# xmed-lab/NEURONS

Measured on AMD Instinct MI355X. Metric: denoising frames/sec, 16f x 256^2 clip, 50 DDIM steps, higher is better.
Workload: dtype bf16; 1 GPU; BASELINE config 2: 1 clip(s) per call, (1,4,16,32,32) latent, 50 DDIM steps, CFG 8.5 (batch 2), SparseCtrl + temporal U-Net per step, random-init weights; clips_per_gpu=5, ddim_steps=50, hip_graph=True, output_finite=True, attention=bf16

## Files before the change

include/neurons_amd.h:

```cpp
#ifndef NEURONS_AMD_H
#define NEURONS_AMD_H

#include <stdint.h>

#ifdef __cplusplus
extern "C" {
#endif

typedef int nr_status;
#define NR_OK 0
#define NR_ERR_ARG 1
#define NR_ERR_STATE 2
#define NR_ERR_MISSING_WEIGHT 3
#define NR_ERR_HIP 4
#define NR_ERR_UNSUPPORTED 5

typedef void* nr_stream;
typedef struct nr_net nr_net;

#define NR_KIND_UNET3D 0
#define NR_KIND_SPARSECTRL 1
#define NR_KIND_SGM_UNET 2

#define NR_KIND_VAE_DECODER 3
// ... 90 lines not shown
                                 double alpha_cumprod_t, double alpha_cumprod_prev, double beta_t);

nr_status nr_cfg_ddim_step(nr_stream stream, const float* eps_dev, const float* x_dev, float* x_out_dev, int64_t n,
                           float guidance_scale, int32_t do_cfg, double alpha_prod_t, double alpha_prod_t_prev);

#define NR_DDIM_EPSILON 0
#define NR_DDIM_SAMPLE 1
#define NR_DDIM_V_PREDICTION 2
nr_status nr_cfg_ddim_step_ex(nr_stream stream, const float* eps_dev, const float* x_dev, float* x_out_dev, float* x0_out_dev, int64_t n,
                              float guidance_scale, int32_t do_cfg, int32_t prediction_type, int32_t clip_sample,
                              int32_t use_clipped_model_output, double alpha_prod_t, double alpha_prod_t_prev, double sigma, double dir_coeff,
                              const float* noise_dev);

nr_status nr_cfg_combine(nr_stream stream, const float* eps_dev, float* eps_out_dev, int64_t n, float guidance_scale);

#define NR_PROF_IGEMM 0
#define NR_PROF_GROUPNORM 1
#define NR_PROF_LAYERNORM 2
#define NR_PROF_ATTENTION 3
#define NR_PROF_OTHER 4
#define NR_PROF_KINDS 5
typedef struct nr_profile {
  double ms[NR_PROF_KINDS];
  double flops[NR_PROF_KINDS];
  double bytes[NR_PROF_KINDS];
  int32_t launches[NR_PROF_KINDS];
} nr_profile;
nr_status nr_net_profile_last(nr_net* h, nr_stream stream, nr_profile* out);

nr_status nr_sparsectrl_forward_async(nr_net* ctrl, nr_stream stream, const float* timesteps, const float* ctx_dev, int32_t ctx_len,
                                      const float* cond_dev, const float* mask_dev, int32_t cond_batch, float scale,
                                      void* const* out_down_dev, void* out_mid_dev, int32_t slot);
nr_status nr_unet3d_forward_after(nr_net* unet, nr_net* ctrl, int32_t slot, nr_stream stream, const float* sample_dev,
                                  const float* timesteps, const float* ctx_dev, int32_t ctx_len, const void* const* down_res_dev,
                                  const void* mid_res_dev, float* out_dev);

nr_status nr_net_set_attention_fp8(nr_net* h, int32_t enable);

nr_status nr_net_set_weight_fp8(nr_net* h, int32_t enable);

nr_status nr_sparsectrl_set_condition_frames(nr_net* h, const int32_t* frames, int32_t n);

nr_status nr_net_set_deterministic_batch(nr_net* h, int32_t enable);
nr_status nr_net_set_clip_samples(nr_net* h, int32_t samples);
nr_status nr_net_set_cfg_pair_identical(nr_net* h, int32_t enable);

int64_t nr_net_export_manifest(nr_net* h, char* buf, int64_t capacity, int64_t* arena_bytes);
nr_status nr_net_export_weights(nr_net* h, nr_stream stream, void* dst_dev, int64_t capacity);
nr_status nr_net_import_weights(nr_net* h, nr_stream stream, const char* manifest, int64_t manifest_bytes, const void* src_dev,
                                int64_t arena_bytes);

nr_status nr_net_set_debug(nr_net* h, int32_t keep_all_activations);
int32_t nr_net_num_taps(const nr_net* h);
const char* nr_net_tap_name(const nr_net* h, int32_t i);
nr_status nr_net_read_tap(nr_net* h, int32_t i, float* host_out, int64_t capacity, int32_t* rows, int32_t* C);

int32_t nr_net_num_ops(const nr_net* h);
const char* nr_net_op_desc(const nr_net* h, int32_t i);

void nr_g8p_set_mode(int32_t mode);
void nr_g8p_set_phases(int32_t phases);
void nr_ff_set_waves(int32_t waves);

nr_status nr_leaf_forward(nr_net* h, nr_stream stream, const float* x_dev, const float* ctx_dev, int32_t ctx_len, float* out_dev);

void nr_op_fm_cache_clear(void);
nr_status nr_op_gemm(nr_stream stream, const void* a_dev, int32_t lda, const void* w_dev, const float* bias_dev,
                     const void* res_dev, int32_t ldr, void* out_dev, int32_t ldo, int32_t M, int32_t N, int32_t K,
                     int32_t geglu);
nr_status nr_op_w8_pack(nr_stream stream, const void* w_dev, int32_t N, int32_t K, void* out_dev, int64_t capacity);
nr_status nr_op_gemm2(nr_stream stream, const void* a0_dev, int32_t c0, int32_t lda0, const void* a1_dev, int32_t c1, int32_t lda1,
                      const void* w_dev, const float* bias_dev, const void* res_dev, int32_t ldr, void* out_dev, int32_t ldo, int32_t M,
                      int32_t N);
nr_status nr_op_ln_gemm(nr_stream stream, const void* a_dev, int32_t lda, const void* w_scaled_dev, const float* ln_c_dev,
                        const float* bias_folded_dev, float eps, const void* res_dev, int32_t ldr, void* out_dev, int32_t ldo,
                        int32_t M, int32_t N, int32_t K, int32_t geglu, int32_t act);
nr_status nr_op_gemm_ex(nr_stream stream, const void* a_dev, int32_t lda, const void* w_dev, const float* bias_dev,
                        const float* ln_c_dev, float ln_eps, const float* rowvec_dev, int32_t rowvec_div, int32_t rowvec_mod,
                        int32_t rowvec_ld, const void* res_dev, int32_t ldr, void* out_dev, int32_t ldo, int32_t M, int32_t N,
                        int32_t K, int32_t geglu, int32_t act, float out_scale);
nr_status nr_op_conv3x3(nr_stream stream, const void* x0_dev, int32_t c0, const void* x1_dev, int32_t c1, int32_t nimg,
                        int32_t H, int32_t W, int32_t stride, int32_t ups, const void* w_dev, const float* bias_dev,
                        const float* rowvec_dev, int32_t rowvec_div, const void* res_dev, void* out_dev, int32_t Cout);
nr_status nr_op_condembed_in(nr_stream stream, const float* cond_dev, const float* mask_dev, int32_t c0, int32_t nsrc, int32_t F, int32_t H,
                             int32_t W, const int32_t* fmap, int32_t nframes, const float* w_dev, const float* bias_dev, int32_t Cout,
                             void* out_dev);
nr_status nr_op_condembed_conv(nr_stream stream, const void* x_dev, int32_t nimg, int32_t H, int32_t W, int32_t Cin, int32_t stride,
                               const void* wfm_dev, const float* bias_dev, int32_t Cout, int32_t silu, void* out_dev);
nr_status nr_op_conv3x3_tap_inner(nr_stream stream, const void* x0, int32_t c0, int32_t nimg, int32_t H, int32_t W, const void* w,
                                  const float* bias, const float* rowvec, int32_t rowvec_div, const void* res, void* out, int32_t Cout);
nr_status nr_op_groupnorm(nr_stream stream, const void* x0_dev, int32_t c0, const void* x1_dev, int32_t c1, int32_t nimg,
                          int32_t hw, int32_t groups, const float* gamma_dev, const float* beta_dev, float eps,
                          int32_t silu, float* partial_ws_dev, void* out_dev);
nr_status nr_op_layernorm(nr_stream stream, const void* x_dev, void* out_dev, int32_t M, int32_t C,
                          const float* gamma_dev, const float* beta_dev, float eps, const float* pe_dev, int32_t pe_hw,
                          int32_t pe_F);
nr_status nr_op_attention(nr_stream stream, int32_t mode, const void* q_dev, const void* kv_dev, void* out_dev,
                          int32_t nimg, int32_t L, int32_t Lk, int32_t C, int32_t heads, int32_t frames, int32_t kv_div);

nr_status nr_op_ff_fused(nr_stream stream, const void* t_dev, const void* x_dev, void* out_dev, int32_t M, int32_t C,
                         const void* w1_geglu_dev, const float* gamma_dev, const float* beta_dev, const float* b1_geglu_dev,
                         const void* wc_dev, const float* bc_dev, float ln_eps);

nr_status nr_op_tattn_fused(nr_stream stream, void* t_dev, int32_t nbatch, int32_t hw, const void* wq_dev, const void* wk_dev,
                            const void* wv_dev, const void* wo_dev, const float* gamma_dev, const float* gb_dev, const float* bo_dev,
                            float ln_eps);
nr_status nr_op_xattn_fused(nr_stream stream, void* t_dev, int32_t nimg, int32_t hw, int32_t img_per_ctx, const void* wq_dev,
                            const void* wo_dev, const void* kv_dev, int32_t ldkv, int32_t Lk, int32_t nctx, const float* gamma_dev,
                            const float* beta_dev, const float* bo_dev, float ln_eps);
nr_status nr_op_tattn_fused_frames(nr_stream stream, void* t_dev, int32_t nbatch, int32_t frames, int32_t hw, const void* wq_dev,
                                   const void* wk_dev, const void* wv_dev, const void* wo_dev, const float* gamma_dev, const float* gb_dev,
                                   const float* bo_dev, float ln_eps);

nr_status nr_op_tattn_head(nr_stream stream, const void* t_dev, void* a_dev, int32_t nbatch, int32_t hw, int32_t C, const void* w_folded_dev,
                           const float* lnc_dev, const float* bias_dev, const float* rowvec_dev, float ln_eps);
nr_status nr_op_tattn_head_frames(nr_stream stream, const void* t_dev, void* a_dev, int32_t nbatch, int32_t frames, int32_t hw, int32_t C,
                                  const void* w_folded_dev, const float* lnc_dev, const float* bias_dev, const float* rowvec_dev, float ln_eps);

nr_status nr_op_xattn_head(nr_stream stream, const void* t_dev, void* a_dev, int32_t nimg, int32_t hw, int32_t img_per_ctx, int32_t C,
                           const void* wq_folded_dev, const float* lnc_dev, const float* bias_dev, const void* kv_dev, int32_t ldkv, int32_t Lk,
                           int32_t nctx, float ln_eps);

#ifdef __cplusplus
}
#endif
#endif
```

neurons_amd/_lib.py:

```python
import ctypes as C
import os

_HERE = os.path.dirname(os.path.abspath(__file__))
LIB_PATH = os.path.join(_HERE, "libneurons_amd" + ("_" + os.environ["NR_LIB_VARIANT"] if os.environ.get("NR_LIB_VARIANT") else "") + ".so")

NR_KIND_UNET3D = 0
NR_KIND_SPARSECTRL = 1
NR_KIND_SGM_UNET = 2
NR_KIND_VAE_DECODER = 3
NR_KIND_VAE_ENCODER = 4
NR_KIND_CLIP_TEXT = 5
NR_KIND_LEAF_TRANSFORMER3D = 6
NR_KIND_LEAF_TEMPORAL = 7
NR_MAX_LEVELS = 4
NR_DDIM_EPSILON = 0
NR_DDIM_SAMPLE = 1
NR_DDIM_V_PREDICTION = 2


class NrNetConfig(C.Structure):
    _fields_ = [
        ("kind", C.c_int32),
        ("in_channels", C.c_int32),
        ("out_channels", C.c_int32),
# ... 11 lines not shown
        ("motion_num_attention_blocks", C.c_int32),
        ("motion_pe_max_len", C.c_int32),
        ("motion_module_mid_block", C.c_int32),
        ("conditioning_channels", C.c_int32),
        ("set_noisy_sample_input_to_zero", C.c_int32),
        ("transformer_depth", C.c_int32 * NR_MAX_LEVELS),
        ("num_head_channels", C.c_int32),
        ("adm_in_channels", C.c_int32),
        ("cond_embedding_levels", C.c_int32),
        ("cond_embedding_channels", C.c_int32 * NR_MAX_LEVELS),
    ]


NR_PROF_KINDS = 5
NR_PROF_NAMES = ("igemm", "groupnorm", "layernorm", "attention", "other")


class NrProfile(C.Structure):
    _fields_ = [("ms", C.c_double * NR_PROF_KINDS), ("flops", C.c_double * NR_PROF_KINDS),
                ("bytes", C.c_double * NR_PROF_KINDS), ("launches", C.c_int32 * NR_PROF_KINDS)]


_VP = C.c_void_p
_FP = C.POINTER(C.c_float)
_I32 = C.c_int32
_I64 = C.c_int64
SYMBOLS = {
    "nr_net_create": (_I32, [C.POINTER(NrNetConfig), C.POINTER(_VP)]),
    "nr_net_destroy": (None, [_VP]),
    "nr_last_error": (C.c_char_p, []),
    "nr_net_load_tensor": (_I32, [_VP, C.c_char_p, _VP, C.POINTER(_I64), _I32]),
    "nr_net_plan": (_I32, [_VP, _I32, _I32, _I32, _I32, _I32]),
    "nr_net_release_host_weights": (_I32, [_VP]),
    "nr_net_invalidate_context": (_I32, [_VP]),
    "nr_net_set_graph": (_I32, [_VP, _I32]),
    "nr_net_workspace_bytes": (_I64, [_VP]),
    "nr_net_weight_bytes": (_I64, [_VP]),
    "nr_net_num_residuals": (_I32, [_VP]),
    "nr_net_residual_shape": (_I32, [_VP, _I32, C.POINTER(_I32), C.POINTER(_I32), C.POINTER(_I32)]),
    "nr_unet3d_forward": (_I32, [_VP, _VP, _VP, _FP, _VP, _I32, C.POINTER(_VP), _VP, _VP]),
    "nr_sparsectrl_forward": (_I32, [_VP, _VP, _VP, _FP, _VP, _I32, _VP, _VP, _I32, C.c_float, C.POINTER(_VP), _VP]),
    "nr_denoise_step_forward": (_I32, [_VP, _VP, _VP, _VP, _FP, _VP, _I32, _VP, _VP, _I32, C.c_float, C.POINTER(_VP), _VP, _VP, _FP]),
    "nr_sparsectrl_forward_async": (_I32, [_VP, _VP, _FP, _VP, _I32, _VP, _VP, _I32, C.c_float, C.POINTER(_VP), _VP, _I32]),
    "nr_unet3d_forward_after": (_I32, [_VP, _VP, _I32, _VP, _VP, _FP, _VP, _I32, C.POINTER(_VP), _VP, _VP]),
    "nr_sgm_unet_forward": (_I32, [_VP, _VP, _VP, C.c_float, _FP, _VP, _I32, _VP, _VP]),
    "nr_vae_decode": (_I32, [_VP, _VP, _VP, C.c_float, C.c_float, C.c_float, _I32, _VP]),
    "nr_clip_text_forward": (_I32, [_VP, _VP, _VP, _VP]),
    "nr_vae_encode": (_I32, [_VP, _VP, _VP, C.c_float, C.c_float, _VP]),
    "nr_gaussian_sample": (_I32, [_VP, _VP, _VP, _VP, _I32, _I32, _I32, C.c_float]),
    "nr_edm_cfg_euler_step": (_I32, [_VP, _VP, _VP, _VP, _I64, C.c_float, C.c_float, C.c_float, C.c_float]),
    "nr_prior_p_sample_step": (_I32, [_VP, _VP, _VP, _VP, _VP, _VP, _VP, _I64, C.c_float, _I32, _I32, C.c_double, C.c_double, C.c_double]),
    "nr_cfg_ddim_step": (_I32, [_VP, _VP, _VP, _VP, _I64, C.c_float, _I32, C.c_double, C.c_double]),
    "nr_cfg_ddim_step_ex": (_I32, [_VP, _VP, _VP, _VP, _VP, _I64, C.c_float, _I32, _I32, _I32, _I32, C.c_double, C.c_double, C.c_double,
                                   C.c_double, _VP]),
    "nr_cfg_combine": (_I32, [_VP, _VP, _VP, _I64, C.c_float]),
    "nr_net_export_manifest": (_I64, [_VP, _VP, _I64, C.POINTER(_I64)]),
    "nr_net_export_weights": (_I32, [_VP, _VP, _VP, _I64]),
    "nr_net_import_weights": (_I32, [_VP, _VP, C.c_char_p, _I64, _VP, _I64]),
    "nr_net_profile_last": (_I32, [_VP, _VP, C.POINTER(NrProfile)]),
    "nr_net_set_attention_fp8": (_I32, [_VP, _I32]),
    "nr_net_set_weight_fp8": (_I32, [_VP, _I32]),
    "nr_net_set_deterministic_batch": (_I32, [_VP, _I32]),
    "nr_net_set_clip_samples": (_I32, [_VP, _I32]),
    "nr_net_set_cfg_pair_identical": (_I32, [_VP, _I32]),
    "nr_sparsectrl_set_condition_frames": (_I32, [_VP, C.POINTER(_I32), _I32]),
    "nr_net_set_debug": (_I32, [_VP, _I32]),
    "nr_net_num_taps": (_I32, [_VP]),
    "nr_net_tap_name": (C.c_char_p, [_VP, _I32]),
    "nr_net_read_tap": (_I32, [_VP, _I32, _VP, _I64, C.POINTER(_I32), C.POINTER(_I32)]),
    "nr_g8p_set_mode": (None, [_I32]),
    "nr_g8p_set_phases": (None, [_I32]),
    "nr_ff_set_waves": (None, [_I32]),
    "nr_net_num_ops": (_I32, [_VP]),
    "nr_net_op_desc": (C.c_char_p, [_VP, _I32]),
    "nr_leaf_forward": (_I32, [_VP, _VP, _VP, _VP, _I32, _VP]),
    "nr_op_fm_cache_clear": (None, []),
    "nr_op_gemm": (_I32, [_VP, _VP, _I32, _VP, _VP, _VP, _I32, _VP, _I32, _I32, _I32, _I32, _I32]),
    "nr_op_w8_pack": (_I32, [_VP, _VP, _I32, _I32, _VP, _I64]),
    "nr_op_gemm2": (_I32, [_VP, _VP, _I32, _I32, _VP, _I32, _I32, _VP, _VP, _VP, _I32, _VP, _I32, _I32, _I32]),
    "nr_op_ln_gemm": (_I32, [_VP, _VP, _I32, _VP, _VP, _VP, C.c_float, _VP, _I32, _VP, _I32, _I32, _I32, _I32, _I32, _I32]),
    "nr_op_gemm_ex": (_I32, [_VP, _VP, _I32, _VP, _VP, _VP, C.c_float, _VP, _I32, _I32, _I32, _VP, _I32, _VP, _I32, _I32, _I32, _I32, _I32, _I32,
                             C.c_float]),
    "nr_op_conv3x3": (_I32, [_VP, _VP, _I32, _VP, _I32, _I32, _I32, _I32, _I32, _I32, _VP, _VP, _VP, _I32, _VP, _VP, _I32]),
    "nr_op_condembed_in": (_I32, [_VP, _VP, _VP, _I32, _I32, _I32, _I32, _I32, C.POINTER(_I32), _I32, _VP, _VP, _I32, _VP]),
    "nr_op_condembed_conv": (_I32, [_VP, _VP, _I32, _I32, _I32, _I32, _I32, _VP, _VP, _I32, _I32, _VP]),
    "nr_op_conv3x3_tap_inner": (_I32, [_VP, _VP, _I32, _I32, _I32, _I32, _VP, _VP, _VP, _I32, _VP, _VP, _I32]),
    "nr_op_groupnorm": (_I32, [_VP, _VP, _I32, _VP, _I32, _I32, _I32, _I32, _VP, _VP, C.c_float, _I32, _VP, _VP]),
    "nr_op_layernorm": (_I32, [_VP, _VP, _VP, _I32, _I32, _VP, _VP, C.c_float, _VP, _I32, _I32]),
    "nr_op_attention": (_I32, [_VP, _I32, _VP, _VP, _VP, _I32, _I32, _I32, _I32, _I32, _I32, _I32]),
    "nr_op_ff_fused": (_I32, [_VP, _VP, _VP, _VP, _I32, _I32, _VP, _VP, _VP, _VP, _VP, _VP, C.c_float]),
    "nr_op_tattn_fused": (_I32, [_VP, _VP, _I32, _I32, _VP, _VP, _VP, _VP, _VP, _VP, _VP, C.c_float]),
    "nr_op_xattn_fused": (_I32, [_VP, _VP, _I32, _I32, _I32, _VP, _VP, _VP, _I32, _I32, _I32, _VP, _VP, _VP, C.c_float]),
    "nr_op_tattn_fused_frames": (_I32, [_VP, _VP, _I32, _I32, _I32, _VP, _VP, _VP, _VP, _VP, _VP, _VP, C.c_float]),
    "nr_op_tattn_head": (_I32, [_VP, _VP, _VP, _I32, _I32, _I32, _VP, _VP, _VP, _VP, C.c_float]),
    "nr_op_tattn_head_frames": (_I32, [_VP, _VP, _VP, _I32, _I32, _I32, _I32, _VP, _VP, _VP, _VP, C.c_float]),
    "nr_op_xattn_head": (_I32, [_VP, _VP, _VP, _I32, _I32, _I32, _I32, _VP, _VP, _VP, _VP, _I32, _I32, _I32, C.c_float]),
}

_lib = None


def load():
    global _lib
    if _lib is not None:
        return _lib
    if not os.path.exists(LIB_PATH):
        raise RuntimeError(
            f"{LIB_PATH} not found: build it with `python -c 'import __graft_entry__ as g; g.build()'` "
            "(make -C neurons_amd/csrc).  neurons_amd has no CPU fallback."
        )
    lib = C.CDLL(LIB_PATH)
    for name, (res, args) in SYMBOLS.items():
        fn = getattr(lib, name)
        fn.restype = res
        fn.argtypes = args
    _lib = lib
    return lib


def check(status):
    if status != 0:
        msg = load().nr_last_error()
        raise RuntimeError(f"neurons_amd: status {status}: {msg.decode() if msg else ''}")
```

neurons_amd/csrc/common.h:

```cpp
#pragma once
#include <hip/hip_runtime.h>
#include <stdint.h>
#include <cmath>
#include <cstring>

typedef __bf16 bf16;
typedef __attribute__((ext_vector_type(8))) __bf16 bf16x8;
typedef __attribute__((ext_vector_type(4))) __bf16 bf16x4;
typedef __attribute__((ext_vector_type(2))) __bf16 bf16x2;
typedef __attribute__((ext_vector_type(4))) float f32x4;

#define NR_WAVE 64

__device__ __forceinline__ float bf2f(bf16 v) { return (float)v; }
__device__ __forceinline__ bf16 f2bf(float v) { return (bf16)v; }

__device__ __forceinline__ bf16x8 bf16x8_zero() {
  bf16x8 z;
#pragma unroll
  for (int i = 0; i < 8; ++i) z[i] = (bf16)0.0f;
  return z;
}

__device__ __forceinline__ float silu_f(float x) { return x * __builtin_amdgcn_rcpf(1.0f + __expf(-x)); }
// ... 76 lines not shown
  p.out_f32 = nr_pin(p.out_f32); p.tap_inner = nr_pin(p.tap_inner); p.w_fm = nr_pin(p.w_fm); p.w8 = nr_pin(p.w8);
  return p;
}

struct NrRowPanelParams {
  const bf16* a; int lda;
  const bf16* w;
  int M, N;
  const float* bias;
  const float* ln_c; float ln_eps;
  const float* rowvec; int rowvec_div, rowvec_mod, rowvec_ld;
  const bf16* res; int ldr;
  bf16* out; int ldo;
  float out_scale; int geglu; int act;
  int nsplit;
};

struct NrAttnParams {
  const bf16* q; const bf16* k; const bf16* v; bf16* out;
  long long q_outer, q_inner_stride, q_seq;
  long long kv_outer, kv_inner_stride, kv_seq;
  long long o_outer, o_inner_stride, o_seq;
  int inner;
  int kv_inner;
  int kv_div;
  int nbatch, heads, d, Lq, Lk;
  float scale;
  int causal;
  int fp8;
};

struct NrGnParams {
  const bf16* x0; const bf16* x1;
  int c0, c1, ld0, ld1;
  int nimg, hw;
  int plan_nimg;
  int groups;
  int pix_per_blk, nchunk;
  float* partial;
  int finalized;
  const float* gamma; const float* beta;
  float eps;
  int silu;
  bf16* out; int ldo;
};

struct NrFfFusedParams {
  const bf16* t; int ldt; const bf16* x; int ldx; bf16* out; int ldo; int M; const bf16* stream; const float *gamma, *beta, *b1, *bc; float ln_eps; int norot, waves; };
struct NrXattnFusedParams {
  bf16* t; int nimg, hw, img_per_ctx, nctx, Lk; const bf16* wstream; const bf16* kvstream; const float *gamma, *beta, *bo; float ln_eps; int norot; };
struct NrTattnFusedParams {
  bf16* t; int nbatch, frames, hw; const bf16* stream; const float *gamma, *gb, *bo; float ln_eps; int norot; };
struct NrXattnHeadParams {
  const bf16* t; bf16* out; int nimg, hw, img_per_ctx, nctx, Lk, C; const bf16* wstream; const bf16* kvstream; const float* table; float ln_eps; };
struct NrTattnHeadParams {
  const bf16* t; bf16* out; int nbatch, frames, hw, C; const bf16* stream; const float* table; float ln_eps; };

struct NrAddMulti {
  bf16* dst[16];
  const bf16* src[16];
  long long n8_end[16];
  int count;
};


inline void nr_conv_out_hw(int H, int W, int ksize, int stride, int ups, int* OH, int* OW) {
  *OH = H; *OW = W;
  if (ksize == 3) {
    if (ups) { *OH *= 2; *OW *= 2; }
    if (stride == 2) { *OH = (*OH - 1) / 2 + 1; *OW = (*OW - 1) / 2 + 1; }
  }
}

inline NrGemmParams nr_gemm_params(const bf16* a0, int c0, int lda0, const bf16* a1, int c1, int lda1, int nimg, int H, int W, int ksize, int stride,
                                   int ups, const bf16* w, int N, const float* bias, const bf16* res, int ldr, bf16* out, int ldo) {
  NrGemmParams p;
  std::memset(&p, 0, sizeof(p));
  p.a0 = a0; p.c0 = c0; p.lda0 = lda0;
  p.a1 = a1; p.c1 = a1 ? c1 : 0; p.lda1 = lda1;
  p.H = H; p.W = W;
  nr_conv_out_hw(H, W, ksize, stride, ups, &p.OH, &p.OW);
  p.ksize = ksize; p.stride = stride; p.ups = ups;
  p.w = w;
  p.M = nimg * p.OH * p.OW; p.N = N; p.K = ksize * ksize * (p.c0 + p.c1);
  p.bias = bias; p.rowvec_div = 1;
  p.res = res; p.ldr = ldr;
  p.out = out; p.ldo = ldo; p.out_scale = 1.f;
  return p;
}

inline NrAttnParams nr_attn_params(int mode, const bf16* q, const bf16* kv, bf16* out, int ldq, int ldkv, int ldo, int nimg, int hw, int Lk, int C,
                                   int heads, int frames, int kv_div, int causal, int fp8) {
  NrAttnParams p;
  std::memset(&p, 0, sizeof(p));
  p.heads = heads; p.d = C / heads; p.scale = 1.0f / std::sqrt((float)p.d);
  p.out = out; p.causal = causal; p.fp8 = fp8;
  if (mode == 0) {
    p.q = q; p.k = q + C; p.v = q + 2 * C;
    p.nbatch = nimg; p.Lq = hw; p.Lk = hw;
    p.inner = 1; p.q_outer = (long long)hw * ldq; p.q_inner_stride = 0; p.q_seq = ldq;
    p.kv_inner = 1; p.kv_outer = p.q_outer; p.kv_inner_stride = 0; p.kv_seq = ldq; p.kv_div = 1;
    p.o_outer = (long long)hw * ldo; p.o_inner_stride = 0; p.o_seq = ldo;
  } else if (mode == 1) {
    p.q = q; p.k = kv; p.v = kv + C;
    p.nbatch = nimg; p.Lq = hw; p.Lk = Lk;
    p.inner = 1; p.q_outer = (long long)hw * ldq; p.q_inner_stride = 0; p.q_seq = ldq;
    p.kv_inner = 1; p.kv_outer = (long long)Lk * ldkv; p.kv_inner_stride = 0; p.kv_seq = ldkv; p.kv_div = kv_div;
    p.o_outer = (long long)hw * ldo; p.o_inner_stride = 0; p.o_seq = ldo;
  } else {
    const int F = frames;
    p.q = q; p.k = q + C; p.v = q + 2 * C;
    p.nbatch = (nimg / F) * hw; p.Lq = F; p.Lk = F;
    p.inner = hw; p.q_outer = (long long)F * hw * ldq; p.q_inner_stride = ldq; p.q_seq = (long long)hw * ldq;
    p.kv_inner = hw; p.kv_outer = p.q_outer; p.kv_inner_stride = ldq; p.kv_seq = p.q_seq; p.kv_div = 1;
    p.o_outer = (long long)F * hw * ldo; p.o_inner_stride = ldo; p.o_seq = (long long)hw * ldo;
  }
  return p;
}

inline NrGnParams nr_gn_params(const bf16* x0, int c0, int ld0, const bf16* x1, int c1, int ld1, int nimg, int hw, int groups, const float* gamma,
                               const float* beta, float eps, int silu, float* partial, bf16* out, int ldo) {
  NrGnParams p;
  std::memset(&p, 0, sizeof(p));
  p.x0 = x0; p.c0 = c0; p.ld0 = ld0;
  p.x1 = x1; p.c1 = x1 ? c1 : 0; p.ld1 = ld1;
  p.nimg = nimg; p.hw = hw; p.groups = groups; p.partial = partial;
  p.gamma = gamma; p.beta = beta; p.eps = eps; p.silu = silu;
  p.out = out; p.ldo = ldo;
  return p;
}
```

neurons_amd/csrc/engine.h:

```cpp
#pragma once
#include "launchers.h"
#include "../../include/neurons_amd.h"

#include <algorithm>
#include <cmath>
#include <cstdio>
#include <cstdlib>
#include <cstring>
#include <functional>
#include <map>
#include <memory>
#include <stdexcept>
#include <string>
#include <vector>

namespace nre {

void set_err(const std::string& s);

struct NrError : std::runtime_error {
  nr_status code;
  NrError(nr_status c, const std::string& m) : std::runtime_error(m), code(c) {}
};

#define HIP_OK(expr)                                                                                        \
  do {                                                                                                      \
    hipError_t _e = (expr);                                                                                 \
    if (_e != hipSuccess) throw nre::NrError(NR_ERR_HIP, std::string(#expr) + ": " + hipGetErrorString(_e)); \
  } while (0)

#define LAUNCH_OK(expr)                                                                                   \
  do {                                                                                                    \
    int _r = (expr);                                                                                      \
    if (_r != 0) throw nre::NrError(NR_ERR_UNSUPPORTED, std::string(#expr) + " -> " + std::to_string(_r)); \
    hipError_t _le = hipGetLastError();                                                                   \
    if (_le != hipSuccess) throw nre::NrError(NR_ERR_HIP, std::string(#expr) + ": " + hipGetErrorString(_le)); \
  } while (0)

#define NR_TRY try {
#define NR_CATCH                                                                   \
  }                                                                                \
  catch (const nre::NrError& e) { nre::set_err(e.what()); return e.code; }         \
  catch (const std::exception& e) { nre::set_err(e.what()); return NR_ERR_STATE; } \
  return NR_OK;

inline float bf2f_host(uint16_t h) {
  const uint32_t u = (uint32_t)h << 16;
  float f;
  std::memcpy(&f, &u, 4);
  return f;
}
inline uint16_t f2bf_host(float f) {
  uint32_t u;
  std::memcpy(&u, &f, 4);
  if ((u & 0x7fffffffu) > 0x7f800000u) return 0x7fc0;
  u += 0x7fffu + ((u >> 16) & 1u);
  return (uint16_t)(u >> 16);
}

template <class... A>
std::string descf(const char* fmt, A... a) { char d[160]; snprintf(d, sizeof(d), fmt, a...); return d; }
inline bool env_is_1(const char* name) {
  const char* v = getenv(name);
  return v && v[0] == '1';
}

struct HostTensor {
  std::vector<float> data;
  std::vector<int64_t> shape;
  int64_t numel() const { int64_t n = 1; for (auto s : shape) n *= s; return n; }
};

struct Arena {
  struct Blk { size_t off, size; };
  std::vector<Blk> free_;
  size_t top = 0, high = 0;
  static size_t align(size_t b) { return (b + 255) & ~(size_t)255; }
  size_t alloc(size_t bytes);
  void release(size_t off, size_t bytes);
  void reset() { free_.clear(); top = 0; high = 0; }
};

struct Buf {
  Arena* arena; size_t off, bytes; bool keep;
  ~Buf() { if (!keep) arena->release(off, bytes); }
};

struct Act {
  std::shared_ptr<Buf> buf;
  bf16* ptr = nullptr;
  int nimg = 0, H = 0, W = 0, C = 0, ld = 0;
  int64_t rows() const { return (int64_t)nimg * H * W; }
  bool valid() const { return nimg > 0; }
};

struct Tap { std::string name; bf16* ptr; int64_t rows; int C, ld; };

struct IO {
  const float* sample;
  const float* ctx;
  float* out;
  const void* down_res[16];
  const void* mid_res;
  int has_res;
  const float* cond;
  const float* mask;
  int cond_batch;
  float scale;
  void* out_down[16];
  void* out_mid;
  const float* y;
  float in_scale;
  const int* ids;
  float in_shift;
  float out_mul, out_add;
  int clamp01;
  bool operator==(const IO& o) const { return std::memcmp(this, &o, sizeof(IO)) == 0; }
};
inline IO new_io() {
  IO io;
  std::memset(&io, 0, sizeof(io));
  io.scale = 1.f; io.in_scale = 1.f; io.out_mul = 1.f; io.cond_batch = 1;
  return io;
}

constexpr int NR_MAX_BATCH = 64;

void launch_copy16(const void* src, void* dst, size_t nbytes, hipStream_t s);

struct TembSlot { std::string prefix; int off, C; };

std::vector<float> sinusoid_table(int max_len, int C);

struct WeightStore {
  const bool& dry;
  explicit WeightStore(const bool& sizing_pass) : dry(sizing_pass) {}
  ~WeightStore();
  WeightStore(const WeightStore&) = delete;

  std::map<std::string, HostTensor> host;
  struct DevW { void* ptr; size_t bytes; };
  std::map<std::string, DevW> dev;
  size_t weight_bytes = 0;
  char* import_base = nullptr;
  size_t import_bytes = 0;
  bool in_import(const void* p) const { return import_base && (const char*)p >= import_base && (const char*)p < import_base + import_bytes; }

  bool load_tensor(const std::string& key, const float* data, const int64_t* shape, int ndim);
  void release_host();
  const HostTensor& need(const std::string& key) const;
  bool has(const std::string& key) const { return host.count(key) != 0; }
  const HostTensor& data_of(const std::string& key) const;
  void check_shape(const std::string& key, const HostTensor& t, std::initializer_list<int64_t> want) const;

  std::string manifest(int kind, size_t* total) const;
  void export_to(void* dst_dev, hipStream_t s) const;
  void import_from(int kind, const std::string& manifest, const void* src_dev, int64_t arena_bytes, hipStream_t s);

  void* upload(const std::string& name, const void* data, size_t bytes);
  void* adopt(const std::string& name, void* d, size_t bytes);
  void erase(const std::string& name);
  std::string name_of(const void* p, const char* who) const;
  template <class Fn>
  void* cached(const std::string& name, Fn make) {
    if (dry) return nullptr;
    auto it = dev.find(name);
    if (it != dev.end()) return it->second.ptr;
    return make();
  }
  template <class Fn>
  void* packed(const std::string& name, size_t bytes, Fn fn, const std::vector<std::string>& inputs = {}) {
    return cached(name, [&]() {
      std::vector<char> had;
      for (auto& in : inputs) had.push_back(dev.count(in) != 0);
      void* d = nullptr;
      HIP_OK(hipMalloc(&d, bytes));
      try { fn(d); HIP_OK(hipDeviceSynchronize()); }
      catch (...) { (void)hipFree(d); throw; }
      adopt(name, d, bytes);
      for (size_t i = 0; i < inputs.size(); ++i) if (!had[i]) erase(inputs[i]);
      return d;
    });
  }
  template <class T, class Fill>
  const T* convert(const char* tag, const std::string& key, std::initializer_list<int64_t> shape, size_t count, Fill fill) {
    check_shape(key, need(key), shape);
    const std::string name = tag + key;
    return (const T*)cached(name, [&]() {
      const HostTensor& t = data_of(key);
      std::vector<T> h(count);
      fill(t.data.data(), h.data());
      return upload(name, h.data(), h.size() * sizeof(T));
    });
  }
  template <class T, class Cvt>
  const T* stacked(const std::string& name, const std::vector<std::string>& keys, Cvt cvt) {
    return (const T*)cached(name, [&]() {
      std::vector<T> h;
      for (auto& k : keys) { const HostTensor& t = data_of(k); for (float f : t.data) h.push_back(cvt(f)); }
      return upload(name, h.data(), h.size() * sizeof(T));
    });
  }

  const bf16* w_linear(const std::string& key, int N, int K);
  const bf16* w_linear_cat(const std::vector<std::string>& keys, int Neach, int K);
  const float* b_cat(const std::vector<std::string>& keys, int Neach);
  struct Stacked { const bf16* w; const float* b; };
  Stacked w_temb_projection(const std::string& tag, const std::vector<TembSlot>& slots, const std::string& layer, int K);
  struct LnW { const bf16* w; const float* c; const float* b; };
  LnW w_ln_linear(const std::vector<std::string>& wkeys, const std::vector<std::string>& bkeys, const std::string& ln, int Neach, int K, bool geglu);
  const float* pe_projection(const std::vector<std::string>& wkeys, int Neach, int K, int max_len);
  struct FoldW { const bf16* w; const float* b; };
  FoldW w_fold_ff_proj(const std::string& ff2, const std::string& po, int C);
  const bf16* w_geglu(const std::string& key, int inner, int K);
  const float* b_geglu(const std::string& key, int inner);
  const bf16* w_conv3(const std::string& key, int Cout, int Cin, bool tap_inner = false);
  const float* w_conv_in(const std::string& key, int Cout, int Cin);
  const bf16* w_condembed(const std::string& key, int Cout, int Cin);
  const float* w_f32_sum(const std::string& a, const std::string& b, int64_t n);
  const float* w_f32(const std::string& key, std::initializer_list<int64_t> shape);
  const float* w_f32(const std::string& key, int64_t n) { return w_f32(key, {n}); }
  const float* pe_table(int C, int max_len);
  const float* b_ln_pe(const std::string& ln, int F, int C);
  const bf16* w_layout(const bf16* w, int N, int K, int layout);

  struct FfFusedW { const bf16* stream; const float *gamma, *beta, *b1, *bc; };
  FfFusedW ff_fused_weights(const std::string& ln, const std::string& ff, const std::string& po, int C);
  struct XattnFusedW { const bf16* wstream; const float *gamma, *beta, *bo; };
  XattnFusedW xattn_fused_weights(const std::string& b, int C);
  struct TattnFusedW { const bf16* stream; const float *gb, *gamma, *bo; };
  TattnFusedW tattn_fused_weights(const std::string& ln, const std::string& ab, int F, int C);
  struct HeadW { const bf16* stream; const float* table; };
  HeadW xattn_head_weights(const std::string& ln, const std::string& wq, int C);
  HeadW tattn_head_weights(const std::string& ln, const std::vector<std::string>& wqkv, int C, int F, int max_len);
  LnW ln_vectors(const std::vector<std::string>& wkeys, const std::string& ln, int Neach, int K);
  const float* fold_bias(const std::string& ff2, const std::string& po, int C);
};

}

struct nr_net {
  using Arena = nre::Arena;
  using Buf = nre::Buf;
  using Act = nre::Act;
  using IO = nre::IO;
  static constexpr int NR_MAX_BATCH = nre::NR_MAX_BATCH;

  nr_net_config cfg;
  int device = -1;

  int B2 = 0, F = 0, H = 0, W = 0, ctx_len = 0;
  bool planned = false;
  bool dry = false;
  nre::WeightStore wts{dry};
  Arena arena;
  Arena parena;
  size_t main_high = 0;
  char* arena_base = nullptr;
  size_t arena_bytes = 0;
  std::vector<std::function<void(hipStream_t)>> ops;
  std::vector<std::function<void(hipStream_t)>> ctx_ops;
  std::vector<Act> ctx_persist;
  bool building_ctx = false;
  bool ctx_dirty = true;
  struct OpMeta { int kind; double flops, bytes; std::string desc; int launches = 1; };
  std::vector<OpMeta> op_meta;
  std::vector<nre::Tap> taps;
  bool keep_all = false;
  bool det_batch = false;
  int clip_samples = 2;
  long long det_rows(long long rows) const {
    if (!det_batch || B2 <= clip_samples) return rows;
    return rows / B2 * clip_samples;
  }
  int n_cond_frames = -1;
  int cond_frames[64] = {0};
  bool cfg_dup = false;
  bool attn_fp8 = false;
  bool w8 = false;
  IO io = nre::new_io();
  int n_res = 0;
  struct ResShape { int C, h, w; };
  std::vector<ResShape> res_shapes;

  float* t_dev = nullptr;
  int temb_total = 0;

  bool use_graph = false;
  struct GraphSlot { IO io = nre::new_io(); hipGraphExec_t exec = nullptr; unsigned long long used = 0; };
  static constexpr int NR_GRAPH_SLOTS = 64;
  std::vector<GraphSlot> gcache[3];
  unsigned long long gclock = 0;
  hipEvent_t ev_slot[2] = {nullptr, nullptr};
  size_t split_op = 0;
  size_t split_op2 = 0;
  hipEvent_t ev_adds = nullptr;
  bool prefetch_valid = false;
  float prefetch_t[NR_MAX_BATCH] = {0};
  IO prefetch_io = nre::new_io();
  hipStream_t own_stream = nullptr;
  hipEvent_t ev_in = nullptr, ev_out = nullptr;

  ~nr_net();

  template <class T>
  T* at(size_t off) const { return reinterpret_cast<T*>(reinterpret_cast<uintptr_t>(arena_base) + off); }
  Act new_act(int nimg, int h, int w, int C) { return act_in(arena, 0, keep_all, nimg, h, w, C); }
  Act new_act_persistent(int nimg, int h, int w, int C) { return act_in(parena, main_high, true, nimg, h, w, C); }
  Act act_in(Arena& a, size_t base, bool keep, int nimg, int h, int w, int C);
  template <class T>
  T* new_scratch(size_t count) { return at<T>(arena.alloc(count * sizeof(T))); }
  std::shared_ptr<Buf> new_tmp(size_t bytes);
  struct SplitK { std::shared_ptr<Buf> buf; float* ws = nullptr; };
  SplitK splitk_scratch(size_t bytes);
  void emit(std::function<void(hipStream_t)> fn, int kind = NR_PROF_OTHER, double flops = 0, double bytes = 0, const std::string& desc = std::string());
  void last_op_launches(int n) { if (!dry && !building_ctx && !op_meta.empty()) op_meta.back().launches = n; }
  void tap(const std::string& name, const Act& a) {
    if (!dry && keep_all) taps.push_back(nre::Tap{name, a.ptr, a.rows(), a.C, a.ld});
  }
  void op_tap(const char* kind, const Act& a);
  void begin_plan();
  Act stage_context();
  Act context_kv(const Act& ctx_bf, const std::string& b, int C, size_t stream_bytes = 0, const std::function<void(const bf16*, int, bf16*, hipStream_t)>& pack = nullptr);

  struct GemmOpt {
    const float* bias = nullptr;
    const float* rowvec = nullptr; int rowvec_div = 1, rowvec_ld = 0, rowvec_mod = 0;
    const Act* res = nullptr;
    float scale = 1.f;
    int geglu = 0;
    Act* out = nullptr;
    int pad_tl0 = 0;
    int act = 0;
    const float* ln_c = nullptr;
    int tap_inner = 0;
    bool derived_w = false;
  };
  Act conv(const Act& x0, const Act* x1, const bf16* w, int Cout, int ksize, int stride, int ups, const GemmOpt& o);
  Act linear(const Act& x, const bf16* w, int N, const GemmOpt& o) { return conv(x, nullptr, w, N, 1, 1, 0, o); }
  Act linear_wb(const Act& x, const std::string& key, int N, const Act* res = nullptr, Act* out = nullptr);
  void gemm_raw(const bf16* a, int lda, const bf16* w, int M, int N, int K, const float* bias, bf16* out, int ldo, float* out32, const char* what);
  Act groupnorm(const Act& x0, const Act* x1, const std::string& prefix, float eps, int silu);
  Act layernorm(const Act& x, const std::string& prefix, const float* pe, int pe_F);
  Act attention(int mode, const Act& q, const Act* kv, int C, int heads, int causal = 0);
  using TembSlot = nre::TembSlot;
  std::vector<TembSlot> temb_slots;
  float* temb_all = nullptr;
  const float* temb_for(const std::string& prefix, int C);
  struct ResKeys { std::string norm1, conv1, norm2, conv2, shortcut; };
  ResKeys res_keys(const std::string& pre) const;
  Act resnet(const Act& x0, const Act* x1, const std::string& pre, int Cout);
  Act ln_linear(const Act& x, const std::string& ln, const std::vector<std::string>& wkeys, const std::vector<std::string>& bkeys, int Neach, bool geglu,
                int act, bool temporal_pe);
  void feed_forward(Act& t, const std::string& ln, const std::string& pre);
  Act feed_forward_proj_out(const Act& x, Act& t, const std::string& ln, const std::string& ff, const std::string& pre);
  bool cfg_dedup_active() const;
  Act expand_cfg(const Act& h);
  enum BlockKernel { BLOCK_UNFUSED, BLOCK_FUSED320, BLOCK_HEAD };
  BlockKernel cross_attn_kernel(const Act& t, int heads, int hw) const;
  BlockKernel temporal_attn_kernel(const Act& t, int heads, int hw) const;
  Act ff_fused_block(const Act& x, const Act& t, const std::string& ln, const std::string& ff, const std::string& po);
  void xattn_fused_block(Act& t, const Act& ctx_bf, const std::string& b, int hw);
  Act xattn_head_block(const Act& t, const Act& ctx_bf, const std::string& b, int hw);
  void tattn_fused_block(Act& t, const std::string& nrm, const std::string& ab, int hw, int heads);
  Act tattn_head_block(const Act& t, const std::string& nrm, const std::vector<std::string>& wqkv, int hw, int heads);
  Act spatial_transformer(const Act& x_in, const Act& ctx_bf, const std::string& pre, int depth = 1, bool cfg_half = false, Act* x_full = nullptr);
  Act temporal_module(const Act& x, const std::string& pre0);
  Act vae_attn(const Act& x, const std::string& pre);

  void enumerate_resnets(std::vector<TembSlot>& out) const;
  struct SgmLayout {
    struct In { int idx; int kind; int level; int Cout; };
    struct Out { int idx; int level; int Cout; bool attn; bool up; };
    std::vector<In> in;
    std::vector<Out> out;
  };
  SgmLayout sgm_layout() const;
  void build_sgm();
  void build_vae();
  void build_vae_enc();
  void build_clip();
  void build_leaf();
  Act embed_conv(const Act& in, int Fe, const std::string& key, int Cout, int stride, int silu, const float* bias);
  void cond_embedding(Act& x, int nd, const int* fmap_reduce, const int* fmap_expand);
  void build();
  void plan(int batch, int frames, int h, int w, int ctxl);

  void drop_graphs();
  void ensure_streams();
  void run_context(hipStream_t s);
  void set_timesteps(hipStream_t s, const float* timesteps);
  void launch_segment(hipStream_t s, int seg);
  void begin(hipStream_t s, const float* timesteps) { set_timesteps(s, timesteps); run_context(s); }
  void run_eager(hipStream_t s, const float* timesteps);
  hipStream_t begin_fenced(hipStream_t caller, const float* timesteps);
  void run(hipStream_t caller, const float* timesteps);
};
```

neurons_amd/csrc/engine_layers.hip:

```cpp
#include "engine.h"

using namespace nre;

size_t Arena::alloc(size_t bytes) {
  bytes = align(bytes);
  for (size_t i = 0; i < free_.size(); ++i) {
    if (free_[i].size >= bytes) {
      const size_t off = free_[i].off;
      if (free_[i].size == bytes) free_.erase(free_.begin() + i);
      else { free_[i].off += bytes; free_[i].size -= bytes; }
      return off;
    }
  }
  const size_t off = top;
  top += bytes;
  if (top > high) high = top;
  return off;
}
void Arena::release(size_t off, size_t bytes) {
  bytes = align(bytes);
  size_t i = 0;
  while (i < free_.size() && free_[i].off < off) ++i;
  free_.insert(free_.begin() + i, Blk{off, bytes});
  if (i + 1 < free_.size() && free_[i].off + free_[i].size == free_[i + 1].off) {
    free_[i].size += free_[i + 1].size;
    free_.erase(free_.begin() + i + 1);
  }
  if (i > 0 && free_[i - 1].off + free_[i - 1].size == free_[i].off) {
    free_[i - 1].size += free_[i].size;
    free_.erase(free_.begin() + i);
  }
  if (!free_.empty() && free_.back().off + free_.back().size == top) {
    top = free_.back().off;
    free_.pop_back();
  }
}

Act nr_net::act_in(Arena& ar, size_t base, bool keep, int nimg, int h, int w, int C) {
  Act a;
  const size_t bytes = (size_t)nimg * h * w * C * sizeof(bf16);
  auto b = std::make_shared<Buf>();
  b->arena = &ar; b->bytes = bytes; b->off = ar.alloc(bytes); b->keep = keep;
  a.buf = b; a.ptr = at<bf16>(base + b->off); a.nimg = nimg; a.H = h; a.W = w; a.C = C; a.ld = C;
  return a;
}
std::shared_ptr<Buf> nr_net::new_tmp(size_t bytes) {
  auto b = std::make_shared<Buf>();
  b->arena = &arena; b->bytes = bytes; b->off = arena.alloc(bytes); b->keep = keep_all;
  return b;
}
nr_net::SplitK nr_net::splitk_scratch(size_t bytes) {
  SplitK k;
  if (bytes) { k.buf = new_tmp(bytes); k.ws = at<float>(k.buf->off); }
  return k;
}
void nr_net::emit(std::function<void(hipStream_t)> fn, int kind, double flops, double bytes, const std::string& desc) {
  if (dry) return;
  if (building_ctx) { ctx_ops.push_back(std::move(fn)); return; }
  ops.push_back(std::move(fn));
  op_meta.push_back(OpMeta{kind, flops, bytes, desc});
}
void nr_net::op_tap(const char* kind, const Act& a) {
  static const bool on = getenv("NR_OP_TAPS") != nullptr;
  if (on && !dry && keep_all && !building_ctx) taps.push_back(Tap{"op" + std::to_string(ops.size()) + "." + kind, a.ptr, a.rows(), a.C, a.ld});
}
void nr_net::begin_plan() {
  ctx_persist.clear(); ops.clear(); ctx_ops.clear(); op_meta.clear(); taps.clear(); arena.reset(); parena.reset();
  ctx_dirty = true;
  temb_slots.clear(); temb_total = 0; temb_all = nullptr;
  n_res = 0; res_shapes.clear();
  t_dev = new_scratch<float>(NR_MAX_BATCH);
}
Act nr_net::stage_context() {
  Act ctx_bf = new_act_persistent(1, 1, B2 * ctx_len, cfg.cross_attention_dim);
  bf16* cp = ctx_bf.ptr; const long long n = (long long)B2 * ctx_len * cfg.cross_attention_dim;
  building_ctx = true;
  emit([this, cp, n](hipStream_t s) { LAUNCH_OK(nr_launch_f32_to_bf16(io.ctx, cp, n, s)); });
  building_ctx = false;
  ctx_persist.push_back(ctx_bf);
  return ctx_bf;
}
Act nr_net::context_kv(const Act& ctx_bf, const std::string& b, int C, size_t stream_bytes, const std::function<void(const bf16*, int, bf16*, hipStream_t)>& pack) {
  building_ctx = true;
  Act kv = new_act_persistent(ctx_bf.nimg, ctx_bf.H, ctx_bf.W, 2 * C);
  GemmOpt ok; ok.out = &kv;
  linear(ctx_bf, wts.w_linear_cat({b + ".attn2.to_k.weight", b + ".attn2.to_v.weight"}, C, cfg.cross_attention_dim), 2 * C, ok);
  Act stream;
  if (pack) {
    stream = new_act_persistent(1, 1, 1, (int)(stream_bytes / sizeof(bf16)));
    const bf16* kvp = kv.ptr; bf16* sp = stream.ptr; const int ldkv = kv.ld;
    emit([=](hipStream_t s) { pack(kvp, ldkv, sp, s); });
  }
  building_ctx = false;
  ctx_persist.push_back(kv);
  if (pack) ctx_persist.push_back(stream);
  return pack ? stream : kv;
}

Act nr_net::conv(const Act& x0, const Act* x1, const bf16* w, int Cout, int ksize, int stride, int ups, const GemmOpt& o) {
  int OH, OW;
  nr_conv_out_hw(x0.H, x0.W, ksize, stride, ups, &OH, &OW);
  const int outC = o.geglu ? Cout / 2 : Cout;
  Act out = o.out ? *o.out : new_act(x0.nimg, OH, OW, outC);
  if (out.C != outC || out.rows() != (int64_t)x0.nimg * OH * OW) throw NrError(NR_ERR_STATE, "conv: output shape mismatch");
  if (o.res && (o.res->C != outC || o.res->rows() != out.rows())) throw NrError(NR_ERR_STATE, "conv: residual shape mismatch");
  NrGemmParams p = nr_gemm_params(x0.ptr, x0.C, x0.ld, x1 ? x1->ptr : nullptr, x1 ? x1->C : 0, x1 ? x1->ld : 0, x0.nimg, x0.H, x0.W, ksize, stride, ups,
                                  w, Cout, o.bias, o.res ? o.res->ptr : nullptr, o.res ? o.res->ld : 0, out.ptr, out.ld);
  p.rowvec = o.rowvec; p.rowvec_div = o.rowvec_div; p.rowvec_ld = o.rowvec_ld; p.rowvec_mod = o.rowvec_mod;
  p.out_scale = o.scale; p.geglu = o.geglu; p.pad_tl0 = o.pad_tl0; p.act = o.act; p.ln_c = o.ln_c; p.ln_eps = 1e-5f;
  p.tap_inner = o.tap_inner;
  p.plan_m = det_batch ? (int)det_rows(p.M) : 0;
  p.w8 = (w8 && ksize == 1 && !o.derived_w) ? 1 : 0;
  NrGemmRoute r;
  LAUNCH_OK(nr_gemm_route(&p, &r));
  const bf16* wk = dry ? reinterpret_cast<const bf16*>(uintptr_t(16)) : wts.w_layout(w, Cout, p.K, r.weight_layout);
  const double in_elems = (double)x0.rows() * (p.c0 + p.c1);
  const double bytes = 2.0 * (in_elems + (double)p.N * p.K + (double)p.M * outC + (o.res ? (double)p.M * outC : 0.0));
  const bool l160 = r.cls == NR_GEMM_LIN160;
  const std::string d = l160 ? descf("%s M=%d N=%d K=%d res=%d geglu=%d ln=%d", r.lin160.form == 4 ? "lin160 panel" : "lin160", p.M, p.N, p.K, o.res ? 1 : 0, p.geglu, p.ln_c ? 1 : 0)
                             : descf("igemm ks=%d s=%d ups=%d M=%d N=%d K=%d geglu=%d res=%d%s", ksize, stride, ups, p.M, p.N, p.K, p.geglu, o.res ? 1 : 0,
                                     r.weight_layout == NR_W_FRAGMAJOR_E4M3 ? " w=e4m3" : "");
  const SplitK sk = splitk_scratch(r.ws_bytes);
  float* ws = sk.ws;
  emit([p, r, wk, ws](hipStream_t s) { LAUNCH_OK(nr_launch_gemm(&p, &r, wk, ws, s)); }, NR_PROF_IGEMM, 2.0 * p.M * (double)p.N * p.K, bytes, d);
  if (ws) last_op_launches(2);
  op_tap(l160 ? "lin160" : (ksize == 3 ? "conv3" : (p.ln_c ? "lngemm" : "gemm")), out);
  return out;
}

Act nr_net::linear_wb(const Act& x, const std::string& key, int N, const Act* res, Act* out) {
  GemmOpt o; o.bias = wts.w_f32(key + ".bias", N); o.res = res; o.out = out;
  return linear(x, wts.w_linear(key + ".weight", N, x.C), N, o);
}

void nr_net::gemm_raw(const bf16* a, int lda, const bf16* w, int M, int N, int K, const float* bias, bf16* out, int ldo, float* out32,
                      const char* what) {
  NrGemmParams p = nr_gemm_params(a, K, lda, nullptr, 0, 0, M, 1, 1, 1, 1, 0, w, N, bias, nullptr, 0, out, ldo);
  p.out_f32 = out32;
  p.plan_m = det_batch ? (int)det_rows(M) : 0;
  NrGemmRoute r;
  LAUNCH_OK(nr_gemm_route_rowmajor(&p, &r));
  const SplitK sk = splitk_scratch(r.ws_bytes);
  float* ws = sk.ws;
  emit([p, r, ws](hipStream_t s) { LAUNCH_OK(nr_launch_gemm(&p, &r, p.w, ws, s)); }, NR_PROF_IGEMM, 2.0 * M * (double)N * K,
       2.0 * ((double)M * K + (double)N * K) + (out32 ? 4.0 : 2.0) * (double)M * N, descf("igemm %s M=%d N=%d K=%d", what, M, N, K));
}

Act nr_net::groupnorm(const Act& x0, const Act* x1, const std::string& prefix, float eps, int silu) {
  const int C = x0.C + (x1 ? x1->C : 0);
  const float* gamma = wts.w_f32(prefix + ".weight", C);
  const float* beta = wts.w_f32(prefix + ".bias", C);
  NrGnParams p = nr_gn_params(x0.ptr, x0.C, x0.ld, x1 ? x1->ptr : nullptr, x1 ? x1->C : 0, x1 ? x1->ld : 0, x0.nimg, x0.H * x0.W, cfg.norm_num_groups, gamma, beta,
                              eps, silu, nullptr, nullptr, C);
  if (x1) p.c1 = x1->C;
  p.plan_nimg = det_batch ? (int)det_rows(x0.nimg) : 0;
  NrGnRoute r;
  LAUNCH_OK(nr_gn_route(&p, &r));
  auto ws = new_tmp((size_t)r.ws_floats * sizeof(float));
  Act out = new_act(x0.nimg, x0.H, x0.W, C);
  p.partial = at<float>(ws->off); p.out = out.ptr;
  if (getenv("NR_OP_TAPS") && keep_all && !x1) {
    Act snap = new_act(x0.nimg, x0.H, x0.W, x0.C);
    const bf16* src = x0.ptr; bf16* dst = snap.ptr; const size_t nb = (size_t)x0.rows() * x0.C * sizeof(bf16);
    if (x0.ld == x0.C) {
      emit([=](hipStream_t s) { launch_copy16(src, dst, nb, s); });
      op_tap("gn_input_snapshot", snap);
    }
  }
  emit([p, r](hipStream_t s) { LAUNCH_OK(nr_launch_groupnorm(&p, &r, s)); }, NR_PROF_GROUPNORM,
       8.0 * (double)x0.rows() * C, 2.0 * 2.0 * (double)x0.rows() * C,
       "groupnorm nimg=" + std::to_string(x0.nimg) + " hw=" + std::to_string(x0.H * x0.W) + " C=" + std::to_string(C));
  last_op_launches(r.launches);
  op_tap("gn", out);
  return out;
}

Act nr_net::layernorm(const Act& x, const std::string& prefix, const float* pe, int pe_F) {
  const float* g = wts.w_f32(prefix + ".weight", x.C);
  const float* b = wts.w_f32(prefix + ".bias", x.C);
  Act out = new_act(x.nimg, x.H, x.W, x.C);
  const bf16* xp = x.ptr; bf16* op = out.ptr;
  const int ldx = x.ld, ldo = out.ld, M = (int)x.rows(), C = x.C, hw = x.H * x.W;
  emit([=](hipStream_t s) { LAUNCH_OK(nr_launch_layernorm(xp, ldx, op, ldo, M, C, g, b, 1e-5f, pe, hw, pe_F, s)); },
       NR_PROF_LAYERNORM, 8.0 * (double)M * C, 2.0 * 2.0 * (double)M * C,
       "layernorm M=" + std::to_string(M) + " C=" + std::to_string(C));
  op_tap("ln", out);
  return out;
}

Act nr_net::attention(int mode, const Act& q, const Act* kv, int C, int heads, int causal) {
  Act out = new_act(q.nimg, q.H, q.W, C);
  const bool vae = cfg.kind == NR_KIND_VAE_DECODER || cfg.kind == NR_KIND_VAE_ENCODER;
  const NrAttnParams p = nr_attn_params(mode, q.ptr, kv ? kv->ptr : nullptr, out.ptr, q.ld, kv ? kv->ld : 0, out.ld, q.nimg, q.H * q.W, ctx_len, C, heads, F,
                                        F, causal, (attn_fp8 && mode != 2 && !vae) ? 1 : 0);
  NrAttnRoute r;
  LAUNCH_OK(nr_attn_route(&p, &r));
  const double flops = 4.0 * (double)p.nbatch * p.heads * (double)p.Lq * p.Lk * p.d;
  const double kvrows = mode == 1 ? (double)(p.nbatch / p.kv_div) * p.Lk : (double)p.nbatch * p.Lk;
  const double bytes = 2.0 * ((double)p.nbatch * p.Lq * C * 2.0 + kvrows * C * 2.0);
  emit([p, r](hipStream_t s) { LAUNCH_OK(nr_launch_attention(&p, &r, s)); }, NR_PROF_ATTENTION, flops, bytes,
       descf("attention mode=%d nbatch=%d heads=%d d=%d Lq=%d Lk=%d", mode, p.nbatch, p.heads, p.d, p.Lq, p.Lk));
  op_tap(mode == 2 ? "tattn" : (mode == 1 ? "xattn" : "sattn"), out);
  return out;
}

const float* nr_net::temb_for(const std::string& prefix, int C) {
  for (auto& s : temb_slots) if (s.prefix == prefix) {
    if (s.C != C) throw NrError(NR_ERR_STATE, "temb slot size mismatch for " + prefix);
    return temb_all + s.off;
  }
// ... 306 lines not shown
```

neurons_amd/csrc/engine_nets.hip:

```cpp
#include "engine.h"

using namespace nre;

void nr_net::enumerate_resnets(std::vector<TembSlot>& out) const {
  int off = 0;
  auto add = [&](const std::string& p, int C) { out.push_back(TembSlot{p, off, C}); off += C; };
  const int L = cfg.num_levels;
  for (int i = 0; i < L; ++i)
    for (int j = 0; j < cfg.layers_per_block; ++j)
      add("down_blocks." + std::to_string(i) + ".resnets." + std::to_string(j), cfg.block_out_channels[i]);
  add("mid_block.resnets.0", cfg.block_out_channels[L - 1]);
  add("mid_block.resnets.1", cfg.block_out_channels[L - 1]);
  if (cfg.kind == NR_KIND_UNET3D)
    for (int i = 0; i < L; ++i)
      for (int j = 0; j < cfg.layers_per_block + 1; ++j)
        add("up_blocks." + std::to_string(i) + ".resnets." + std::to_string(j), cfg.block_out_channels[L - 1 - i]);
}

nr_net::SgmLayout nr_net::sgm_layout() const {
  SgmLayout l;
  const int L = cfg.num_levels;
  int idx = 0;
  l.in.push_back({idx++, 0, 0, cfg.block_out_channels[0]});
  for (int lev = 0; lev < L; ++lev) {
// ... 16 lines not shown
  if (F != 1) throw NrError(NR_ERR_ARG, "sgm UNetModel is a 2-D network: plan with frames = 1");
  const SgmLayout lay = sgm_layout();
  begin_plan();
  {
    int off = 0;
    auto add = [&](const std::string& p, int C) { temb_slots.push_back(TembSlot{p, off, C}); off += C; };
    for (auto& b : lay.in) if (b.kind == 1) add("input_blocks." + std::to_string(b.idx) + ".0", b.Cout);
    add("middle_block.0", cfg.block_out_channels[L - 1]);
    add("middle_block.2", cfg.block_out_channels[L - 1]);
    for (auto& b : lay.out) add("output_blocks." + std::to_string(b.idx) + ".0", b.Cout);
    temb_total = off;
  }
  float* sincos = new_scratch<float>((size_t)B2 * C0);
  float* e1 = new_scratch<float>((size_t)B2 * temb_dim);
  float* et = new_scratch<float>((size_t)B2 * temb_dim);
  float* y1 = new_scratch<float>((size_t)B2 * temb_dim);
  float* emb = new_scratch<float>((size_t)B2 * temb_dim);
  temb_all = new_scratch<float>((size_t)B2 * temb_total);
  {
    const int adm = cfg.adm_in_channels;
    const bf16* w1 = wts.w_linear("time_embed.0.weight", temb_dim, C0);
    const float* b1 = wts.w_f32("time_embed.0.bias", temb_dim);
    const bf16* w2 = wts.w_linear("time_embed.2.weight", temb_dim, temb_dim);
    const float* b2 = wts.w_f32("time_embed.2.bias", temb_dim);
    const bf16* wy1 = wts.w_linear("label_emb.0.0.weight", temb_dim, adm);
    const float* by1 = wts.w_f32("label_emb.0.0.bias", temb_dim);
    const bf16* wy2 = wts.w_linear("label_emb.0.2.weight", temb_dim, temb_dim);
    const float* by2 = wts.w_f32("label_emb.0.2.bias", temb_dim);
    const auto proj = wts.w_temb_projection("sgm", temb_slots, ".emb_layers.1", temb_dim);
    const bf16* wp = proj.w; const float* bp = proj.b;
    float* td = t_dev; float* ta = temb_all;
    const int b2n = B2, tt = temb_total;
    emit([=, this](hipStream_t s) {
      LAUNCH_OK(nr_launch_timestep_sincos(td, b2n, C0, sincos, s));
      LAUNCH_OK(nr_launch_linear_small(sincos, b2n, C0, w1, b1, temb_dim, 0, 1, e1, nullptr, s));
      LAUNCH_OK(nr_launch_linear_small(e1, b2n, temb_dim, w2, b2, temb_dim, 0, 0, et, nullptr, s));
      LAUNCH_OK(nr_launch_linear_small(io.y, b2n, adm, wy1, by1, temb_dim, 0, 1, y1, nullptr, s));
      LAUNCH_OK(nr_launch_linear_small(y1, b2n, temb_dim, wy2, by2, temb_dim, 0, 1, emb, et, s));
      LAUNCH_OK(nr_launch_linear_small(emb, b2n, temb_dim, wp, bp, tt, 0, 0, ta, nullptr, s));
    });
    last_op_launches(6);
  }
  Act ctx_bf = stage_context();
  std::vector<Act> hs;
  Act x;
  for (auto& b : lay.in) {
    const std::string bp = "input_blocks." + std::to_string(b.idx);
    if (b.kind == 0) {
      x = new_act(nimg, H, W, C0);
      const float* wT = wts.w_conv_in(bp + ".0.weight", C0, cfg.in_channels);
      const float* bi = wts.w_f32(bp + ".0.bias", C0);
      bf16* xp = x.ptr; const int ic = cfg.in_channels, b2n = B2, Hn = H, Wn = W;
      emit([=, this](hipStream_t s) {
        LAUNCH_OK(nr_launch_conv_in_small(io.sample, nullptr, ic, 0, b2n, nimg, 1, Hn, Wn, wT, bi, nullptr, C0, xp, io.in_scale, 0.f, s));
      });
      tap(bp, x);
    } else if (b.kind == 1) {
      x = resnet(x, nullptr, bp + ".0", b.Cout);
      if (cfg.down_block_has_attn[b.level]) x = spatial_transformer(x, ctx_bf, bp + ".1", cfg.transformer_depth[b.level]);
    } else {
      GemmOpt o; o.bias = wts.w_f32(bp + ".0.op.bias", b.Cout);
      x = conv(x, nullptr, wts.w_conv3(bp + ".0.op.weight", b.Cout, b.Cout), b.Cout, 3, 2, 0, o);
      tap(bp, x);
    }
    hs.push_back(x);
  }
  {
    const int Cm = cfg.block_out_channels[L - 1];
    x = resnet(x, nullptr, "middle_block.0", Cm);
    x = spatial_transformer(x, ctx_bf, "middle_block.1", cfg.transformer_depth[L - 1]);
    x = resnet(x, nullptr, "middle_block.2", Cm);
  }
  for (auto& b : lay.out) {
    const std::string bp = "output_blocks." + std::to_string(b.idx);
    Act skip = hs.back();
    hs.pop_back();
    x = resnet(x, &skip, bp + ".0", b.Cout);
    skip = Act();
    int sub = 1;
    if (b.attn) { x = spatial_transformer(x, ctx_bf, bp + ".1", cfg.transformer_depth[b.level]); sub = 2; }
    if (b.up) {
      const std::string up = bp + "." + std::to_string(sub) + ".conv";
      GemmOpt o; o.bias = wts.w_f32(up + ".bias", b.Cout);
      x = conv(x, nullptr, wts.w_conv3(up + ".weight", b.Cout, b.Cout), b.Cout, 3, 1, 1, o);
      tap(bp + "." + std::to_string(sub), x);
    }
  }
  Act hn = groupnorm(x, nullptr, "out.0", cfg.norm_eps, 1);
  {
    const bf16* wo = wts.w_conv3("out.2.weight", cfg.out_channels, C0);
    const float* bo = wts.w_f32("out.2.bias", cfg.out_channels);
    const bf16* hp = hn.ptr; const int Hn = H, Wn = W, oc = cfg.out_channels;
    emit([=, this](hipStream_t s) { LAUNCH_OK(nr_launch_conv_out_small(hp, C0, nimg, 1, Hn, Wn, wo, bo, oc, io.out, 1.f, 0.f, 0, s)); });
  }
}

void nr_net::build_vae() {
  const int L = cfg.num_levels, zc = cfg.in_channels, nimg = B2;
  if (F != 1) throw NrError(NR_ERR_ARG, "the VAE decoder is a 2-D network: plan with frames = 1");
  begin_plan();
  const int Cm = cfg.block_out_channels[L - 1];
  float* zq = new_scratch<float>((size_t)nimg * zc * H * W);
  {
    const float* Q = wts.w_f32("post_quant_conv.weight", {zc, zc});
    const float* qb = wts.w_f32("post_quant_conv.bias", zc);
    const int hw = H * W;
    emit([=, this](hipStream_t s) { LAUNCH_OK(nr_launch_post_quant(io.sample, io.in_scale, Q, qb, zq, nimg, zc, hw, s)); });
  }
  Act x = new_act(nimg, H, W, Cm);
  {
    const float* wT = wts.w_conv_in("decoder.conv_in.weight", Cm, zc);
    const float* bi = wts.w_f32("decoder.conv_in.bias", Cm);
    bf16* xp = x.ptr; const int Hn = H, Wn = W;
    emit([=](hipStream_t s) {
      LAUNCH_OK(nr_launch_conv_in_small(zq, nullptr, zc, 0, nimg, nimg, 1, Hn, Wn, wT, bi, nullptr, Cm, xp, 1.f, 0.f, s));
    });
    tap("decoder.conv_in", x);
  }
  x = resnet(x, nullptr, "decoder.mid.block_1", Cm);
  x = vae_attn(x, "decoder.mid.attn_1");
  x = resnet(x, nullptr, "decoder.mid.block_2", Cm);
  for (int lev = L - 1; lev >= 0; --lev) {
    const int Co = cfg.block_out_channels[lev];
    const std::string up = "decoder.up." + std::to_string(lev);
    for (int j = 0; j < cfg.layers_per_block + 1; ++j) x = resnet(x, nullptr, up + ".block." + std::to_string(j), Co);
    if (lev != 0) {
      GemmOpt o; o.bias = wts.w_f32(up + ".upsample.conv.bias", Co);
      x = conv(x, nullptr, wts.w_conv3(up + ".upsample.conv.weight", Co, Co), Co, 3, 1, 1, o);
      tap(up + ".upsample", x);
    }
  }
  Act hn = groupnorm(x, nullptr, "decoder.norm_out", cfg.norm_eps, 1);
  {
    const int C0 = cfg.block_out_channels[0], oc = cfg.out_channels;
    const bf16* wo = wts.w_conv3("decoder.conv_out.weight", oc, C0);
    const float* bo = wts.w_f32("decoder.conv_out.bias", oc);
    const bf16* hp = hn.ptr; const int Hn = x.H, Wn = x.W;
    emit([=, this](hipStream_t s) { LAUNCH_OK(nr_launch_conv_out_small(hp, C0, nimg, 1, Hn, Wn, wo, bo, oc, io.out, io.out_mul, io.out_add, io.clamp01, s)); });
  }
}


void nr_net::build_vae_enc() {
  const int L = cfg.num_levels, zc2 = cfg.out_channels, nimg = B2, ic = cfg.in_channels;
  if (F != 1) throw NrError(NR_ERR_ARG, "the VAE encoder is a 2-D network: plan with frames = 1");
  begin_plan();
  const int C0 = cfg.block_out_channels[0];
  Act x = new_act(nimg, H, W, C0);
  {
    const float* wT = wts.w_conv_in("encoder.conv_in.weight", C0, ic);
    const float* bi = wts.w_f32("encoder.conv_in.bias", C0);
    bf16* xp = x.ptr; const int Hn = H, Wn = W;
    emit([=, this](hipStream_t s) {
      LAUNCH_OK(nr_launch_conv_in_small(io.sample, nullptr, ic, 0, nimg, nimg, 1, Hn, Wn, wT, bi, nullptr, C0, xp, io.in_scale,
                                        io.in_shift, s));
    });
    tap("encoder.conv_in", x);
  }
  for (int lev = 0; lev < L; ++lev) {
    const int Co = cfg.block_out_channels[lev];
    const std::string dn = "encoder.down." + std::to_string(lev);
    for (int j = 0; j < cfg.layers_per_block; ++j) x = resnet(x, nullptr, dn + ".block." + std::to_string(j), Co);
    if (lev != L - 1) {
      GemmOpt o; o.bias = wts.w_f32(dn + ".downsample.conv.bias", Co); o.pad_tl0 = 1;
      x = conv(x, nullptr, wts.w_conv3(dn + ".downsample.conv.weight", Co, Co), Co, 3, 2, 0, o);
      tap(dn + ".downsample", x);
    }
  }
  const int Cm = cfg.block_out_channels[L - 1];
  x = resnet(x, nullptr, "encoder.mid.block_1", Cm);
  x = vae_attn(x, "encoder.mid.attn_1");
  x = resnet(x, nullptr, "encoder.mid.block_2", Cm);
  Act hn = groupnorm(x, nullptr, "encoder.norm_out", cfg.norm_eps, 1);
  {
    const int hw = x.H * x.W;
    float* mraw = new_scratch<float>((size_t)nimg * zc2 * hw);
    const bf16* wo = wts.w_conv3("encoder.conv_out.weight", zc2, Cm);
    const float* bo = wts.w_f32("encoder.conv_out.bias", zc2);
    const float* Q = wts.w_f32("quant_conv.weight", {zc2, zc2});
    const float* qb = wts.w_f32("quant_conv.bias", zc2);
    const bf16* hp = hn.ptr; const int Hn = x.H, Wn = x.W;
    emit([=, this](hipStream_t s) {
      LAUNCH_OK(nr_launch_conv_out_small(hp, Cm, nimg, 1, Hn, Wn, wo, bo, zc2, mraw, 1.f, 0.f, 0, s));
      LAUNCH_OK(nr_launch_post_quant(mraw, 1.f, Q, qb, io.out, nimg, zc2, hw, s));
    });
  }
}


void nr_net::build_clip() {
  const int C = cfg.block_out_channels[0], heads = cfg.num_heads, inter = cfg.cross_attention_dim, vocab = cfg.in_channels;
  const int L = W, M = B2 * L;
  if (F != 1 || H != 1) throw NrError(NR_ERR_ARG, "CLIP text encoder: plan with frames = 1, h = 1, w = sequence length");
  if (L > cfg.motion_pe_max_len) throw NrError(NR_ERR_ARG, "sequence longer than max_position_embeddings");
  begin_plan();
  const std::string tm = "text_model.";
  Act x = new_act(B2, 1, L, C);
  {
    const std::string tk = tm + "embeddings.token_embedding.weight", pk = tm + "embeddings.position_embedding.weight";
    const float* tok = wts.w_f32(tk, {vocab, C});
    const float* pos = wts.w_f32(pk, {cfg.motion_pe_max_len, C});
    bf16* xp = x.ptr;
    emit([=, this](hipStream_t s) { LAUNCH_OK(nr_launch_clip_embed(io.ids, tok, pos, xp, M, L, C, vocab, s)); });
    tap("text_model.embeddings", x);
  }
  for (int i = 0; i < cfg.layers_per_block; ++i) {
    const std::string lp = tm + "encoder.layers." + std::to_string(i);
    const std::string ap = lp + ".self_attn";
    Act qkv = ln_linear(x, lp + ".layer_norm1", {ap + ".q_proj.weight", ap + ".k_proj.weight", ap + ".v_proj.weight"},
                        {ap + ".q_proj.bias", ap + ".k_proj.bias", ap + ".v_proj.bias"}, C, false, 0, false);
    Act ao = attention(0, qkv, nullptr, C, heads, 1);
// ... 262 lines not shown
  {
    const int Cm = cfg.block_out_channels[L - 1];
    x = resnet(x, nullptr, "mid_block.resnets.0", Cm);
    x = spatial_transformer(x, ctx_bf, "mid_block.attentions.0");
    if (cfg.use_motion_module && cfg.motion_module_mid_block) x = temporal_module(x, "mid_block.motion_modules.0");
    x = resnet(x, nullptr, "mid_block.resnets.1", Cm);
  }
  res_shapes.push_back(ResShape{x.C, x.H, x.W});
  mid_in = Act();

  if (cfg.kind == NR_KIND_SPARSECTRL) {
    for (int i = 0; i <= n_res; ++i) {
      const bool is_mid = i == n_res;
      const Act& src = is_mid ? x : skips[i];
      const std::string key = is_mid ? std::string("controlnet_mid_block") : "controlnet_down_blocks." + std::to_string(i);
      const bf16* w = wts.w_linear(key + ".weight", src.C, src.C);
      const float* bias = wts.w_f32(key + ".bias", src.C);
      NrGemmParams p = nr_gemm_params(src.ptr, src.C, src.ld, nullptr, 0, 0, src.nimg, src.H, src.W, 1, 1, 0, w, src.C, bias, nullptr, 0, nullptr, src.C);
      p.plan_m = det_batch ? (int)det_rows(p.M) : 0;
      NrGemmRoute r;
      LAUNCH_OK(nr_gemm_route_rowmajor(&p, &r));
      const SplitK sk = splitk_scratch(r.ws_bytes);
      float* ws = sk.ws;
      emit([this, p, r, i, is_mid, ws](hipStream_t s) {
        NrGemmParams q = p;
        q.out = (bf16*)(is_mid ? io.out_mid : io.out_down[i]);
        q.out_scale = io.scale;
        LAUNCH_OK(nr_launch_gemm(&q, &r, q.w, ws, s));
      }, NR_PROF_IGEMM, 2.0 * p.M * (double)p.N * p.K, 2.0 * (2.0 * p.M * (double)p.N + (double)p.N * p.K));
    }
    return;
  }

  split_op = ops.size();
  {
    struct AddT { bf16* dst; long long n; };
    std::vector<AddT> adds;
    for (int i = 0; i < n_res; ++i) adds.push_back(AddT{skips[i].ptr, (long long)skips[i].rows() * skips[i].C});
    adds.push_back(AddT{x.ptr, (long long)x.rows() * x.C});
    bool multi = (int)adds.size() <= 16;
    for (auto& a : adds) multi = multi && a.n % 8 == 0;
    if (multi) {
      NrAddMulti am;
      std::memset(&am, 0, sizeof(am));
      long long acc = 0;
      for (size_t i = 0; i < adds.size(); ++i) { am.dst[i] = adds[i].dst; acc += adds[i].n / 8; am.n8_end[i] = acc; }
      am.count = (int)adds.size();
      const int nr = n_res;
      emit([this, am, nr](hipStream_t st) {
        if (!io.has_res) return;
        NrAddMulti q = am;
        for (int i = 0; i < nr; ++i) q.src[i] = (const bf16*)io.down_res[i];
        q.src[nr] = (const bf16*)io.mid_res;
        LAUNCH_OK(nr_launch_add_bf16_multi(&q, st));
      });
    } else {
      for (int i = 0; i < n_res; ++i) {
        bf16* sp = adds[i].dst; const long long n = adds[i].n;
        emit([this, sp, n, i](hipStream_t st) {
          if (io.has_res) LAUNCH_OK(nr_launch_add_bf16(sp, (const bf16*)io.down_res[i], sp, n, st));
        });
      }
      bf16* xp = x.ptr; const long long n = adds.back().n;
      emit([this, xp, n](hipStream_t st) {
        if (io.has_res) LAUNCH_OK(nr_launch_add_bf16(xp, (const bf16*)io.mid_res, xp, n, st));
      });
    }
  }
  split_op2 = ops.size();

  for (int i = 0; i < L; ++i) {
    const int Cout = cfg.block_out_channels[L - 1 - i];
    const std::string bp = "up_blocks." + std::to_string(i);
    for (int j = 0; j < cfg.layers_per_block + 1; ++j) {
      Act skip = skips.back();
      skips.pop_back();
      x = resnet(x, &skip, bp + ".resnets." + std::to_string(j), Cout);
      skip = Act();
      if (cfg.up_block_has_attn[i]) x = spatial_transformer(x, ctx_bf, bp + ".attentions." + std::to_string(j));
      if (cfg.use_motion_module) x = temporal_module(x, bp + ".motion_modules." + std::to_string(j));
    }
    if (i != L - 1) {
      GemmOpt o; o.bias = wts.w_f32(bp + ".upsamplers.0.conv.bias", Cout);
      x = conv(x, nullptr, wts.w_conv3(bp + ".upsamplers.0.conv.weight", Cout, Cout), Cout, 3, 1, 1, o);
      tap(bp + ".upsamplers.0", x);
    }
  }

  Act hn = groupnorm(x, nullptr, "conv_norm_out", cfg.norm_eps, 1);
  {
    const bf16* wo = wts.w_conv3("conv_out.weight", cfg.out_channels, C0);
    const float* bo = wts.w_f32("conv_out.bias", cfg.out_channels);
    const bf16* hp = hn.ptr; const int Fn = F, Hn = H, Wn = W, oc = cfg.out_channels;
    emit([=, this](hipStream_t s) { LAUNCH_OK(nr_launch_conv_out_small(hp, C0, nimg, Fn, Hn, Wn, wo, bo, oc, io.out, 1.f, 0.f, 0, s)); });
  }
}

void nr_net::plan(int batch, int frames, int h, int w, int ctxl) {
  const bool leaf = cfg.kind == NR_KIND_LEAF_TRANSFORMER3D || cfg.kind == NR_KIND_LEAF_TEMPORAL;
  const bool vae = cfg.kind == NR_KIND_VAE_DECODER || cfg.kind == NR_KIND_VAE_ENCODER || cfg.kind == NR_KIND_CLIP_TEXT || cfg.kind == NR_KIND_LEAF_TEMPORAL;
  if (batch <= 0 || batch > NR_MAX_BATCH || frames <= 0 || h <= 0 || w <= 0 || (ctxl <= 0 && !vae)) throw NrError(NR_ERR_ARG, "plan: bad shape");
  const int down = (cfg.kind == NR_KIND_VAE_DECODER || cfg.kind == NR_KIND_CLIP_TEXT || leaf) ? 1 : 1 << (cfg.num_levels - 1);
  if (h % down != 0 || w % down != 0)
    throw NrError(NR_ERR_ARG, "plan: latent h,w must be multiples of " + std::to_string(down));
  HIP_OK(hipDeviceSynchronize());
  drop_graphs();
  B2 = batch; F = frames; H = h; W = w; ctx_len = ctxl;
  planned = false;
  dry = true;
  char* old = arena_base; arena_base = nullptr;
  main_high = 0;
  try { build(); }
  catch (...) { dry = false; arena_base = old; throw; }
  main_high = Arena::align(arena.high + 256);
  const size_t need_bytes = main_high + parena.high + 256;
  dry = false;
  arena_base = old;
  if (need_bytes > arena_bytes) {
    if (arena_base) { HIP_OK(hipFree(arena_base)); arena_base = nullptr; }
    HIP_OK(hipMalloc((void**)&arena_base, need_bytes));
    arena_bytes = need_bytes;
  }
  split_op = 0; split_op2 = 0;
  prefetch_valid = false;
  build();
  if (split_op == 0 || split_op > ops.size()) split_op = ops.size();
  if (split_op2 < split_op || split_op2 > ops.size()) split_op2 = ops.size();
  HIP_OK(hipDeviceSynchronize());
  planned = true;
}
```

neurons_amd/csrc/engine_ops.hip:

```cpp
#include "engine.h"
#include <tuple>

using namespace nre;

struct OpScratch { void* ptr = nullptr; size_t cap = 0; };
static bool op_scratch(OpScratch& b, size_t need) {
  if (need <= b.cap) return false;
  if (b.ptr) { HIP_OK(hipDeviceSynchronize()); (void)hipFree(b.ptr); }
  b.ptr = nullptr; b.cap = 0;
  HIP_OK(hipMalloc(&b.ptr, need));
  b.cap = need;
  return true;
}

static std::map<std::tuple<const void*, int, int, int>, bf16*> g_op_fm_cache;
extern "C" void nr_op_fm_cache_clear() {
  (void)hipDeviceSynchronize();
  for (auto& kv : g_op_fm_cache) (void)hipFree(kv.second);
  g_op_fm_cache.clear();
}
static const bf16* op_pack(const NrGemmParams& p, const NrGemmRoute& r, hipStream_t s) {
  if (r.weight_layout == NR_W_ROWMAJOR || r.weight_layout == NR_W_TAP_INNER) return p.w;
  const size_t need = nr_gemm_packed_bytes(r.weight_layout, p.N, p.K);
  if (!need) throw NrError(NR_ERR_STATE, "op_pack: shape has no packed form");
// ... 6 lines not shown
      it = g_op_fm_cache.emplace(std::make_tuple(p.w, r.weight_layout, p.N, p.K), d).first;
    }
    return it->second;
  }
  static OpScratch scratch[2];
  OpScratch& b = scratch[(r.weight_layout == NR_W_FRAGMAJOR || r.weight_layout == NR_W_FRAGMAJOR_E4M3) ? 0 : 1];
  op_scratch(b, need);
  LAUNCH_OK(nr_launch_gemm_w_pack(r.weight_layout, p.w, p.N, p.K, (bf16*)b.ptr, s));
  return (const bf16*)b.ptr;
}
static void op_gemm(const NrGemmParams& p_arg, hipStream_t s) {
  NrGemmParams p = p_arg;
  p.w8 = env_is_1("NR_W8") ? 1 : 0;
  NrGemmRoute r;
  LAUNCH_OK(nr_gemm_route(&p, &r));
  const bf16* wk = op_pack(p, r, s);
  static OpScratch ws;
  op_scratch(ws, r.ws_bytes);
  LAUNCH_OK(nr_launch_gemm(&p, &r, wk, r.ws_bytes ? (float*)ws.ptr : nullptr, s));
}

extern "C" nr_status nr_op_gemm(nr_stream stream, const void* a, int32_t lda, const void* w, const float* bias,
                                const void* res, int32_t ldr, void* out, int32_t ldo, int32_t M, int32_t N, int32_t K,
                                int32_t geglu) {
  NR_TRY
  NrGemmParams p = nr_gemm_params((const bf16*)a, K, lda, nullptr, 0, 0, M, 1, 1, 1, 1, 0, (const bf16*)w, N, bias, (const bf16*)res, ldr, (bf16*)out, ldo);
  p.geglu = geglu;
  op_gemm(p, (hipStream_t)stream);
  NR_CATCH
}

extern "C" nr_status nr_op_w8_pack(nr_stream stream, const void* w_dev, int32_t N, int32_t K, void* out_dev, int64_t capacity) {
  NR_TRY
  if (!w_dev || !out_dev) throw NrError(NR_ERR_ARG, "null argument");
  const size_t need = nr_gemm_packed_bytes(NR_W_FRAGMAJOR_E4M3, N, K);
  if (!need) throw NrError(NR_ERR_ARG, "e4m3 weights: N must be a multiple of 16 and K of 64");
  if (capacity < (int64_t)need) throw NrError(NR_ERR_ARG, "output buffer too small");
  LAUNCH_OK(nr_launch_gemm_w_pack(NR_W_FRAGMAJOR_E4M3, (const bf16*)w_dev, N, K, (bf16*)out_dev, (hipStream_t)stream));
  NR_CATCH
}

extern "C" nr_status nr_op_gemm2(nr_stream stream, const void* a0, int32_t c0, int32_t lda0, const void* a1, int32_t c1, int32_t lda1,
                                 const void* w, const float* bias, const void* res, int32_t ldr, void* out, int32_t ldo, int32_t M, int32_t N) {
  NR_TRY
  NrGemmParams p = nr_gemm_params((const bf16*)a0, c0, lda0, (const bf16*)a1, c1, lda1, M, 1, 1, 1, 1, 0, (const bf16*)w, N, bias, (const bf16*)res, ldr,
                                  (bf16*)out, ldo);
  op_gemm(p, (hipStream_t)stream);
  NR_CATCH
}

extern "C" nr_status nr_op_ln_gemm(nr_stream stream, const void* a, int32_t lda, const void* w_scaled, const float* ln_c,
                                   const float* bias_folded, float eps, const void* res, int32_t ldr, void* out, int32_t ldo,
                                   int32_t M, int32_t N, int32_t K, int32_t geglu, int32_t act) {
  NR_TRY
  if (!ln_c) throw NrError(NR_ERR_ARG, "ln_c is required");
  NrGemmParams p = nr_gemm_params((const bf16*)a, K, lda, nullptr, 0, 0, M, 1, 1, 1, 1, 0, (const bf16*)w_scaled, N, bias_folded, (const bf16*)res, ldr,
                                  (bf16*)out, ldo);
  p.geglu = geglu; p.ln_c = ln_c; p.ln_eps = eps; p.act = act;
  op_gemm(p, (hipStream_t)stream);
  NR_CATCH
}

extern "C" nr_status nr_op_gemm_ex(nr_stream stream, const void* a, int32_t lda, const void* w, const float* bias, const float* ln_c,
                                   float ln_eps, const float* rowvec, int32_t rowvec_div, int32_t rowvec_mod, int32_t rowvec_ld,
                                   const void* res, int32_t ldr, void* out, int32_t ldo, int32_t M, int32_t N, int32_t K, int32_t geglu,
                                   int32_t act, float out_scale) {
  NR_TRY
  NrGemmParams p = nr_gemm_params((const bf16*)a, K, lda, nullptr, 0, 0, M, 1, 1, 1, 1, 0, (const bf16*)w, N, bias, (const bf16*)res, ldr, (bf16*)out, ldo);
  p.out_scale = out_scale; p.geglu = geglu; p.act = act;
  p.rowvec = rowvec; p.rowvec_div = rowvec_div > 0 ? rowvec_div : 1; p.rowvec_mod = rowvec_mod; p.rowvec_ld = rowvec_ld;
  p.ln_c = ln_c; p.ln_eps = ln_eps;
  op_gemm(p, (hipStream_t)stream);
  NR_CATCH
}

extern "C" nr_status nr_op_conv3x3(nr_stream stream, const void* x0, int32_t c0, const void* x1, int32_t c1, int32_t nimg,
                                   int32_t H, int32_t W, int32_t stride, int32_t ups, const void* w, const float* bias,
                                   const float* rowvec, int32_t rowvec_div, const void* res, void* out, int32_t Cout) {
  NR_TRY
  NrGemmParams p = nr_gemm_params((const bf16*)x0, c0, c0, (const bf16*)x1, c1, c1, nimg, H, W, 3, stride, ups, (const bf16*)w, Cout, bias, (const bf16*)res,
                                  Cout, (bf16*)out, Cout);
  p.rowvec = rowvec; p.rowvec_div = rowvec_div > 0 ? rowvec_div : 1; p.rowvec_ld = Cout;
  op_gemm(p, (hipStream_t)stream);
  NR_CATCH
}

extern "C" nr_status nr_op_condembed_in(nr_stream stream, const float* cond, const float* mask, int32_t c0, int32_t nsrc, int32_t F, int32_t H,
                                        int32_t W, const int32_t* fmap, int32_t nframes, const float* w, const float* bias, int32_t Cout,
                                        void* out) {
  NR_TRY
  if (!fmap) throw NrError(NR_ERR_ARG, "fmap is null");
  LAUNCH_OK(nr_launch_condembed_in(cond, mask, c0, nsrc, F, H, W, fmap, nframes, w, bias, Cout, (bf16*)out, (hipStream_t)stream));
  NR_CATCH
}

extern "C" nr_status nr_op_condembed_conv(nr_stream stream, const void* x, int32_t nimg, int32_t H, int32_t W, int32_t Cin, int32_t stride,
                                          const void* wfm, const float* bias, int32_t Cout, int32_t silu, void* out) {
  NR_TRY
  LAUNCH_OK(nr_launch_condembed_conv((const bf16*)x, nimg, H, W, Cin, stride, (const bf16*)wfm, bias, Cout, silu, (bf16*)out,
                                     (hipStream_t)stream));
  NR_CATCH
}

extern "C" nr_status nr_op_conv3x3_tap_inner(nr_stream stream, const void* x0, int32_t c0, int32_t nimg, int32_t H, int32_t W, const void* w,
                                             const float* bias, const float* rowvec, int32_t rowvec_div, const void* res, void* out,
                                             int32_t Cout) {
  NR_TRY
  NrGemmParams p = nr_gemm_params((const bf16*)x0, c0, c0, nullptr, 0, 0, nimg, H, W, 3, 1, 0, (const bf16*)w, Cout, bias, (const bf16*)res, Cout, (bf16*)out,
                                  Cout);
  p.tap_inner = 1;
  p.rowvec = rowvec; p.rowvec_div = rowvec_div > 0 ? rowvec_div : 1; p.rowvec_ld = Cout;
  op_gemm(p, (hipStream_t)stream);
  NR_CATCH
}

extern "C" nr_status nr_op_groupnorm(nr_stream stream, const void* x0, int32_t c0, const void* x1, int32_t c1, int32_t nimg,
                                     int32_t hw, int32_t groups, const float* gamma, const float* beta, float eps,
                                     int32_t silu, float* partial_ws, void* out) {
  NR_TRY
  NrGnParams p = nr_gn_params((const bf16*)x0, c0, c0, (const bf16*)x1, c1, c1, nimg, hw, groups, gamma, beta, eps, silu, partial_ws, (bf16*)out,
                              c0 + (x1 ? c1 : 0));
  NrGnRoute r;
  if (const int rc = nr_gn_route(&p, &r)) throw NrError(NR_ERR_UNSUPPORTED, "nr_gn_route -> " + std::to_string(rc) + ": no kernel serves this shape, nr_launch_groupnorm not called");
  LAUNCH_OK(nr_launch_groupnorm(&p, &r, (hipStream_t)stream));
  NR_CATCH
}

extern "C" nr_status nr_op_layernorm(nr_stream stream, const void* x, void* out, int32_t M, int32_t C, const float* gamma,
                                     const float* beta, float eps, const float* pe, int32_t pe_hw, int32_t pe_F) {
  NR_TRY
  LAUNCH_OK(nr_launch_layernorm((const bf16*)x, C, (bf16*)out, C, M, C, gamma, beta, eps, pe, pe_hw > 0 ? pe_hw : 1,
                                pe_F > 0 ? pe_F : 1, (hipStream_t)stream));
  NR_CATCH
}

extern "C" nr_status nr_op_attention(nr_stream stream, int32_t mode, const void* qp, const void* kvp, void* outp,
                                     int32_t nimg, int32_t L, int32_t Lk, int32_t C, int32_t heads, int32_t frames,
                                     int32_t kv_div) {
  NR_TRY
  const int fp8_flag = (mode & 8) ? 1 : 0;
  const int causal_flag = (mode & 16) ? 1 : 0;
  mode &= 7;
  if (causal_flag && (mode != 0 || fp8_flag)) throw NrError(NR_ERR_ARG, "causal attention: mode 0 only");
  if (mode > 2) throw NrError(NR_ERR_ARG, "bad attention mode");
  const NrAttnParams p = nr_attn_params(mode, (const bf16*)qp, (const bf16*)kvp, (bf16*)outp, mode == 1 ? C : 3 * C, 2 * C, C, nimg, L, Lk, C, heads, frames, kv_div,
                                        causal_flag, fp8_flag);
  NrAttnRoute r;
  if (const int rc = nr_attn_route(&p, &r)) throw NrError(NR_ERR_UNSUPPORTED, "nr_attn_route -> " + std::to_string(rc) + ": no kernel serves this shape, nr_launch_attention not called");
  LAUNCH_OK(nr_launch_attention(&p, &r, (hipStream_t)stream));
  NR_CATCH
}

template <class T> static T* op_packed(OpScratch& b, size_t bytes) { op_scratch(b, bytes); return (T*)b.ptr; }

extern "C" nr_status nr_op_ff_fused(nr_stream stream, const void* t_dev, const void* x_dev, void* out_dev, int32_t M, int32_t C, const void* w1_geglu_dev,
                                    const float* gamma_dev, const float* beta_dev, const float* b1_geglu_dev, const void* wc_dev, const float* bc_dev, float ln_eps) {
  NR_TRY
  if (!nr_ff_fused_supported(C, C, C, C)) throw NrError(NR_ERR_UNSUPPORTED, "the fused FeedForward kernel is built for C = 320");
  static OpScratch buf;
  bf16* ws = op_packed<bf16>(buf, nr_ff_stream_bytes(C));
  if (w1_geglu_dev) LAUNCH_OK(nr_launch_ff_stream_pack((const bf16*)w1_geglu_dev, (const bf16*)wc_dev, ws, (hipStream_t)stream));
  const NrFfFusedParams p{.t = (const bf16*)t_dev, .ldt = C, .x = (const bf16*)x_dev, .ldx = C, .out = (bf16*)out_dev, .ldo = C, .M = M, .stream = ws, .gamma = gamma_dev,
                          .beta = beta_dev, .b1 = b1_geglu_dev, .bc = bc_dev, .ln_eps = ln_eps, .norot = env_is_1("NR_DETERMINISTIC_BATCH"), .waves = nr_ff_waves()};
  LAUNCH_OK(nr_launch_ff_fused(&p, (hipStream_t)stream));
  NR_CATCH
}
// ... 88 lines not shown
```

neurons_amd/csrc/engine_weights.hip:

```cpp
#include "engine.h"

namespace nre {

std::vector<float> sinusoid_table(int max_len, int C) {
  std::vector<float> h((size_t)max_len * C);
  const float k = (float)(-std::log(10000.0) / (double)C);
  for (int pos = 0; pos < max_len; ++pos)
    for (int i = 0; i < C; i += 2) {
      const float a = (float)pos * std::exp((float)i * k);
      h[(size_t)pos * C + i] = std::sin(a);
      if (i + 1 < C) h[(size_t)pos * C + i + 1] = std::cos(a);
    }
  return h;
}

static int geglu_src_row(int n, int inner) {
  const int q = n / 32, j = n % 32;
  return j < 16 ? q * 16 + j : inner + q * 16 + (j - 16);
}

static const char* const TAG_LIN = "lin:";
static const char* const TAG_GEGLU = "geglu:";
static std::string ln_name(char part, const std::vector<std::string>& wkeys, const std::vector<std::string>& bkeys, const std::string& ln) {
  std::string name = std::string("ln") + part + ":" + ln + "|";
// ... 237 lines not shown
  r.c = (const float*)upload(nc, hc.data(), hc.size() * 4);
  r.b = (const float*)upload(nb, hb.data(), hb.size() * 4);
  return r;
}
const float* WeightStore::pe_projection(const std::vector<std::string>& wkeys, int Neach, int K, int max_len) {
  std::string name = "perv:" + std::to_string(max_len) + ":";
  for (auto& k : wkeys) name += k + "|";
  return (const float*)cached(name, [&]() {
    const size_t N = (size_t)Neach * wkeys.size();
    const std::vector<float> pe = sinusoid_table(max_len, K);
    std::vector<float> rv((size_t)max_len * N);
    for (size_t mi = 0; mi < wkeys.size(); ++mi) {
      const HostTensor& W = data_of(wkeys[mi]);
      for (int n = 0; n < Neach; ++n)
        for (int f = 0; f < max_len; ++f) {
          double a = 0.0;
          const float* wr = W.data.data() + (size_t)n * K;
          const float* pr = pe.data() + (size_t)f * K;
          for (int k = 0; k < K; ++k) a += (double)pr[k] * (double)wr[k];
          rv[(size_t)f * N + mi * Neach + n] = (float)a;
        }
    }
    return upload(name, rv.data(), rv.size() * 4);
  });
}
WeightStore::FoldW WeightStore::w_fold_ff_proj(const std::string& ff2, const std::string& po, int C) {
  const int J = 4 * C;
  check_shape(ff2 + ".weight", need(ff2 + ".weight"), {C, J});
  check_shape(ff2 + ".bias", need(ff2 + ".bias"), {C});
  check_shape(po + ".weight", need(po + ".weight"), {C, C});
  check_shape(po + ".bias", need(po + ".bias"), {C});
  FoldW r{nullptr, nullptr};
  if (dry) return r;
  const std::string nw = fold_name('w', ff2, po), nb = fold_name('b', ff2, po);
  auto it = dev.find(nw), itb = dev.find(nb);
  if (it != dev.end() && itb != dev.end()) return FoldW{(const bf16*)it->second.ptr, (const float*)itb->second.ptr};
  if (itb != dev.end()) erase(nb);
  const HostTensor& W2 = data_of(po + ".weight");
  const HostTensor& B2 = data_of(po + ".bias");
  const HostTensor& W1 = data_of(ff2 + ".weight");
  const HostTensor& B1 = data_of(ff2 + ".bias");
  const size_t wcb = (size_t)C * (C + J) * sizeof(bf16), bcb = (size_t)C * sizeof(float);
  r.w = (const bf16*)packed(nw, wcb, [&](void* dwc) {
    float *dw2 = nullptr, *dw1 = nullptr, *db2 = nullptr, *db1 = nullptr;
    void* dbc = nullptr;
    HIP_OK(hipMalloc(&dw2, W2.data.size() * 4)); HIP_OK(hipMalloc(&dw1, W1.data.size() * 4));
    HIP_OK(hipMalloc(&db2, B2.data.size() * 4)); HIP_OK(hipMalloc(&db1, B1.data.size() * 4));
    HIP_OK(hipMalloc(&dbc, bcb));
    HIP_OK(hipMemcpy(dw2, W2.data.data(), W2.data.size() * 4, hipMemcpyHostToDevice));
    HIP_OK(hipMemcpy(dw1, W1.data.data(), W1.data.size() * 4, hipMemcpyHostToDevice));
    HIP_OK(hipMemcpy(db2, B2.data.data(), B2.data.size() * 4, hipMemcpyHostToDevice));
    HIP_OK(hipMemcpy(db1, B1.data.data(), B1.data.size() * 4, hipMemcpyHostToDevice));
    LAUNCH_OK(nr_launch_fold_linear_pair(dw2, dw1, db2, db1, C, J, (bf16*)dwc, (float*)dbc, nullptr));
    HIP_OK(hipDeviceSynchronize());
    (void)hipFree(dw2); (void)hipFree(dw1); (void)hipFree(db2); (void)hipFree(db1);
    r.b = (const float*)adopt(nb, dbc, bcb);
  });
  return r;
}
const bf16* WeightStore::w_geglu(const std::string& key, int inner, int K) {
  return (const bf16*)convert<uint16_t>(TAG_GEGLU, key, {2 * inner, K}, (size_t)2 * inner * K, [&](const float* s, uint16_t* h) {
    for (int n = 0; n < 2 * inner; ++n) {
      const int src = geglu_src_row(n, inner);
      for (int k = 0; k < K; ++k) h[(size_t)n * K + k] = f2bf_host(s[(size_t)src * K + k]);
    }
  });
}
const float* WeightStore::b_geglu(const std::string& key, int inner) {
  return convert<float>("geglub:", key, {2 * inner}, (size_t)2 * inner, [&](const float* s, float* h) {
    for (int n = 0; n < 2 * inner; ++n) h[n] = s[geglu_src_row(n, inner)];
  });
}
const bf16* WeightStore::w_conv3(const std::string& key, int Cout, int Cin, bool tap_inner) {
  if (tap_inner && Cin % 64 != 0) throw NrError(NR_ERR_UNSUPPORTED, "tap-inner conv layout needs Cin % 64 == 0: " + key);
  return (const bf16*)convert<uint16_t>(tap_inner ? "conv3t:" : "conv3:", key, {Cout, Cin, 3, 3}, (size_t)Cout * 9 * Cin, [&](const float* s, uint16_t* h) {
    for (int o = 0; o < Cout; ++o)
      for (int c = 0; c < Cin; ++c)
        for (int k = 0; k < 9; ++k) {
          const size_t dst = tap_inner ? (size_t)(c / 64) * 9 * 64 + (size_t)k * 64 + (c % 64) : (size_t)k * Cin + c;
          h[(size_t)o * 9 * Cin + dst] = f2bf_host(s[((size_t)o * Cin + c) * 9 + k]);
        }
  });
}
const float* WeightStore::w_conv_in(const std::string& key, int Cout, int Cin) {
  return convert<float>("convin:", key, {Cout, Cin, 3, 3}, (size_t)Cin * 9 * Cout, [&](const float* s, float* h) {
    for (int o = 0; o < Cout; ++o)
      for (int k = 0; k < Cin * 9; ++k) h[(size_t)k * Cout + o] = s[(size_t)o * Cin * 9 + k];
  });
}
const bf16* WeightStore::w_condembed(const std::string& key, int Cout, int Cin) {
  return (const bf16*)convert<uint16_t>("cefm:", key, {Cout, Cin, 3, 3}, (size_t)nr_condembed_wfm_elems(Cin, Cout), [&](const float* s, uint16_t* h) {
    const int K = 9 * Cin, KS = (K + 31) / 32;
    for (int T = 0; T < Cout / 16; ++T)
      for (int ks = 0; ks < KS; ++ks)
        for (int lane = 0; lane < 64; ++lane)
          for (int j = 0; j < 8; ++j) {
            const int o = 16 * T + (lane & 15), k = 32 * ks + 8 * (lane >> 4) + j;
            if (k >= K) continue;
            const int tap = k / Cin, c = k % Cin;
            h[(((size_t)T * KS + ks) * 64 + lane) * 8 + j] = f2bf_host(s[((size_t)o * Cin + c) * 9 + tap]);
          }
  });
}
const float* WeightStore::w_f32_sum(const std::string& a, const std::string& b, int64_t n) {
  check_shape(a, need(a), {n});
  check_shape(b, need(b), {n});
  const std::string name = "f32sum:" + a + "|" + b;
  return (const float*)cached(name, [&]() {
    const HostTensor& ta = data_of(a);
    const HostTensor& tb = data_of(b);
    std::vector<float> h((size_t)n);
    for (int64_t i = 0; i < n; ++i) h[i] = ta.data[i] + tb.data[i];
    return upload(name, h.data(), h.size() * 4);
  });
}
const float* WeightStore::w_f32(const std::string& key, std::initializer_list<int64_t> shape) {
  check_shape(key, need(key), shape);
  return (const float*)cached("f32:" + key, [&]() { const HostTensor& t = data_of(key); return upload("f32:" + key, t.data.data(), t.data.size() * 4); });
}
const float* WeightStore::pe_table(int C, int max_len) {
  const std::string name = "pe:" + std::to_string(C) + ":" + std::to_string(max_len);
  return (const float*)cached(name, [&]() {
    const std::vector<float> h = sinusoid_table(max_len, C);
    return upload(name, h.data(), h.size() * 4);
  });
}
const float* WeightStore::b_ln_pe(const std::string& ln, int F, int C) {
  check_shape(ln + ".bias", need(ln + ".bias"), {C});
  const std::string name = "tagb:" + std::to_string(F) + ":" + ln;
  return (const float*)cached(name, [&]() {
    const HostTensor& be = data_of(ln + ".bias");
    std::vector<float> h = sinusoid_table(F, C);
    for (int pos = 0; pos < F; ++pos)
      for (int i = 0; i < C; ++i) h[(size_t)pos * C + i] = be.data[i] + h[(size_t)pos * C + i];
    return upload(name, h.data(), h.size() * 4);
  });
}

WeightStore::LnW WeightStore::ln_vectors(const std::vector<std::string>& wkeys, const std::string& ln, int Neach, int K) {
  auto ic = dev.find(ln_name('c', wkeys, {}, ln)), ib = dev.find(ln_name('b', wkeys, {}, ln));
  if (!dry && ic != dev.end() && ib != dev.end()) return LnW{nullptr, (const float*)ic->second.ptr, (const float*)ib->second.ptr};
  return w_ln_linear(wkeys, {}, ln, Neach, K, false);
}
const float* WeightStore::fold_bias(const std::string& ff2, const std::string& po, int C) {
  auto ib = dev.find(fold_name('b', ff2, po));
  return (!dry && ib != dev.end()) ? (const float*)ib->second.ptr : w_fold_ff_proj(ff2, po, C).b;
}
WeightStore::FfFusedW WeightStore::ff_fused_weights(const std::string& ln, const std::string& ff, const std::string& po, int C) {
  const int inner = 4 * C;
  const std::string w1 = ff + ".net.0.proj.weight", ff2 = ff + ".net.2";
  check_shape(w1, need(w1), {2 * inner, C});
  FfFusedW r{};
  r.b1 = b_geglu(ff + ".net.0.proj.bias", inner); r.gamma = w_f32(ln + ".weight", C); r.beta = w_f32(ln + ".bias", C);
  bool packed_now = false;
  r.stream = (const bf16*)packed("ffs:" + w1 + "|" + ff2 + ".weight|" + ff2 + ".bias|" + po + ".weight|" + po + ".bias", nr_ff_stream_bytes(C), [&](void* d) {
    const bf16* wg = w_geglu(w1, inner, C);
    LAUNCH_OK(nr_launch_ff_stream_pack(wg, w_fold_ff_proj(ff2, po, C).w, (bf16*)d, nullptr));
    packed_now = true;
  }, {TAG_GEGLU + w1});
  if (packed_now) erase(fold_name('w', ff2, po));
  r.bc = fold_bias(ff2, po, C);
  return r;
}
WeightStore::XattnFusedW WeightStore::xattn_fused_weights(const std::string& b, int C) {
  const std::string wq = b + ".attn2.to_q.weight", wo = b + ".attn2.to_out.0.weight";
  for (auto& k : {wq, wo}) check_shape(k, need(k), {C, C});
// ... 43 lines not shown
```

neurons_amd/csrc/gemm.hip:

```cpp
#include "launchers.h"
#include "device_prims.h"
#include <cstdio>
#include <cstdlib>

namespace {

__device__ __forceinline__ void glds16_builtin(const void* src, void* lds_wave_base) {
  __builtin_amdgcn_global_load_lds((gptr_t)src, (lptr_t)lds_wave_base, 16, 0, 0);
}

NR_STAMP_BUF(nr_stamp_buf, 512, 48);
#define NR_STAMP_AT(slot) NR_STAMP_PUT(nr_stamp_buf, slot)
#define NR_STAMP_RT(slot) NR_STAMP_PUT_RT(nr_stamp_buf, slot)

template <int BM, int BN, int NS, int WGM, int WGN, bool LNF = false, bool ADMA = false, bool LIN = LNF>
__global__ __launch_bounds__(64 * WGM * WGN, (LNF && WGM * WGN == 8) ? 4 : 1) void igemm_bf16_kernel(NrGemmParams p_arg, int splitk, float* partial, int m_fast) {
  NrGemmParams p = nr_pin_params(p_arg);
  if constexpr (LIN) { p.ksize = 1; p.stride = 1; p.ups = 0; p.a1 = nullptr; p.c1 = 0; p.tap_inner = 0; p.pad_tl0 = 0; }
  splitk = nr_pin(splitk); partial = nr_pin(partial); m_fast = nr_pin(m_fast);
  constexpr int BK = 64;
  constexpr int NW = WGM * WGN;
  constexpr int WM = BM / WGM, WN = BN / WGN;
  constexpr int MT = WM / 16, NT = WN / 16;
  constexpr int GA = BM / (8 * NW), GB = BN / (8 * NW);
  static_assert(BM % (8 * NW) == 0 && BN % (8 * NW) == 0, "tile rows must split evenly over the waves");
  constexpr int TILE = (BM + BN) * BK;
  extern __shared__ __attribute__((aligned(16))) bf16 smem[];

  const int tid = threadIdx.x;
  const int lane = tid & 63;
  const int wave = tid >> 6;
  NR_STAMP_AT(0);
  NR_STAMP_RT(44);
  const int wm = wave / WGN, wn = wave % WGN;
  const int ntn = (p.N + BN - 1) / BN;
  const int ntm = (p.M + BM - 1) / BM;
  int bid;
  {
    const int nwg = gridDim.x, orig = blockIdx.x;
    const int q = nwg >> 3, r = nwg & 7, xcd = orig & 7, local = orig >> 3;
    bid = (xcd < r ? xcd * (q + 1) : r * (q + 1) + (xcd - r) * q) + local;
  }
  const int slice = splitk > 1 ? nr_fdiv_small(bid, ntn * ntm) : 0;
  bid -= slice * ntn * ntm;
  int bm, bn;
  if (m_fast >= 2) {
    const int G = m_fast;
    const int band = nr_fdiv_small(bid, G * ntn);
    const int first = band * G;
    const int gsz = min(G, ntm - first);
    const int r = bid - band * G * ntn;
    bn = nr_fdiv_small(r, gsz);
    bm = first + r - bn * gsz;
  } else if (m_fast) { bn = nr_fdiv_small(bid, ntm); bm = bid - bn * ntm; } else { bm = nr_fdiv_small(bid, ntn); bn = bid - bm * ntn; }
  const int m0 = bm * BM, n0 = bn * BN;
  NR_STAMP_AT(40);
  const int lr = lane >> 3;
  const int lp = lane & 7;
  const int lchunk = (lp ^ lr) << 3;

  const int Cin = p.c0 + p.c1;

  int a_pix[GA], a_oy[GA], a_ox[GA];
  bool a_ok[GA];
#pragma unroll
  for (int j = 0; j < GA; ++j) {
    const int m = m0 + 8 * (wave * GA + j) + lr;
    a_ok[j] = m < p.M;
    const int mm = a_ok[j] ? m : 0;
    if (p.ksize == 1) {
      a_pix[j] = mm; a_oy[j] = 0; a_ox[j] = 0;
    } else {
      const int ohw = p.OH * p.OW;
      const int n = nr_fdiv_small(mm, ohw);
      const int r = mm - n * ohw;
      a_pix[j] = n; a_oy[j] = nr_fdiv_small(r, p.OW); a_ox[j] = r - a_oy[j] * p.OW;
    }
  }
  const bf16* zsrc = (const bf16*)nr_zero16;
  const bool tap_inner = !LNF && p.tap_inner != 0;
  long long a_cbyte[GA];
  unsigned a_tapmask[GA];
  if (tap_inner) {
#pragma unroll
    for (int j = 0; j < GA; ++j) {
      a_cbyte[j] = (((long long)a_pix[j] * p.H + a_oy[j]) * p.W + a_ox[j]) * p.lda0 * (long long)sizeof(bf16);
      unsigned msk = 0;
#pragma unroll
      for (int t = 0; t < 9; ++t) {
        const int iy = a_oy[j] + t / 3 - 1, ix = a_ox[j] + t % 3 - 1;
        if (a_ok[j] && iy >= 0 && iy < p.H && ix >= 0 && ix < p.W) msk |= 1u << t;
      }
      a_tapmask[j] = msk;
    }
  }

  NR_STAMP_AT(41);
  const int nk_total = p.K / BK;
  int kt_begin = 0, kt_end = nk_total;
  if (splitk > 1) { kt_begin = nr_fdiv_small(nk_total * slice, splitk); kt_end = nr_fdiv_small(nk_total * (slice + 1), splitk); }

  const bf16* ap[GA];
  int ainc[GA];
  const bf16* wp[GB];
  int winc[GB];
  int st_tap, st_c;
  {
    const int kbase = kt_begin * BK;
    if (tap_inner) { const int q9 = nr_fdiv_small(kt_begin, 9); st_tap = kt_begin - 9 * q9; st_c = q9 * BK; }
    else { st_tap = p.ksize == 3 ? nr_fdiv_small(kbase, Cin) : 0; st_c = kbase - st_tap * Cin; }
#pragma unroll
    for (int j = 0; j < GB; ++j) {
      const int n = n0 + 8 * (wave * GB + j) + lr;
      const bool ok = n < p.N;
      wp[j] = ok ? p.w + (size_t)n * p.K + kbase + lchunk : zsrc;
      winc[j] = ok ? BK : 0;
    }
  }
  auto setup_rows_tap_inner = [&]() {
    const int ky = st_tap / 3, kx = st_tap - ky * 3;
    const long long delta = ((long long)(ky - 1) * p.W + (kx - 1)) * p.lda0 * (long long)sizeof(bf16);
    const char* base = reinterpret_cast<const char*>(p.a0 + st_c + lchunk) + delta;
#pragma unroll
    for (int j = 0; j < GA; ++j) {
      const bool ok = (a_tapmask[j] >> st_tap) & 1u;
      ap[j] = ok ? reinterpret_cast<const bf16*>(base + a_cbyte[j]) : zsrc;
    }
  };
  auto setup_rows = [&]() {
    if (tap_inner) { setup_rows_tap_inner(); return; }
    const bf16* src; int ld;
    if (st_c < p.c0) { src = p.a0 + st_c; ld = p.lda0; } else { src = p.a1 + (st_c - p.c0); ld = p.lda1; }
    src += lchunk;
    if (p.ksize == 1) {
#pragma unroll
      for (int j = 0; j < GA; ++j) {
        ap[j] = a_ok[j] ? src + (size_t)a_pix[j] * ld : zsrc;
        ainc[j] = a_ok[j] ? BK : 0;
      }
    } else {
      const int ky = st_tap / 3, kx = st_tap - ky * 3;
      const int VH = p.ups ? p.H * 2 : p.H, VW = p.ups ? p.W * 2 : p.W;
#pragma unroll
      for (int j = 0; j < GA; ++j) {
        int iy = a_oy[j] * p.stride + ky - (p.pad_tl0 ? 0 : 1);
        int ix = a_ox[j] * p.stride + kx - (p.pad_tl0 ? 0 : 1);
        const bool ok = a_ok[j] && iy >= 0 && iy < VH && ix >= 0 && ix < VW;
        if (p.ups) { iy >>= 1; ix >>= 1; }
        const size_t pix = ((size_t)a_pix[j] * p.H + iy) * p.W + ix;
        ap[j] = ok ? src + pix * ld : zsrc;
        ainc[j] = ok ? BK : 0;
      }
    }
  };
  NR_STAMP_AT(42);
  setup_rows();
  NR_STAMP_AT(43);

  auto stage = [&](int buf) {
    bf16* sA = smem + buf * TILE;
    bf16* sB = sA + BM * BK;
    if constexpr (ADMA) {
      const unsigned la = nr_lds_addr(sA + wave * GA * 8 * BK), lb = nr_lds_addr(sB + wave * GB * 8 * BK);
#pragma unroll
      for (int j = 0; j < GA; ++j) nr_glds16(ap[j], la + (unsigned)(j * 8 * BK * (int)sizeof(bf16)));
#pragma unroll
      for (int j = 0; j < GB; ++j) nr_glds16(wp[j], lb + (unsigned)(j * 8 * BK * (int)sizeof(bf16)));
    } else {
#pragma unroll
      for (int j = 0; j < GA; ++j) glds16_builtin(ap[j], sA + (wave * GA + j) * 8 * BK);
#pragma unroll
      for (int j = 0; j < GB; ++j) glds16_builtin(wp[j], sB + (wave * GB + j) * 8 * BK);
    }
#pragma unroll
    for (int j = 0; j < GB; ++j) wp[j] += winc[j];
    if (tap_inner) {
      st_tap += 1;
      if (st_tap == 9) { st_tap = 0; st_c += BK; }
      setup_rows_tap_inner();
      return;
    }
    st_c += BK;
    bool resetup = false;
    if (st_c == Cin) { st_c = 0; st_tap += 1; resetup = true; }
    else if (p.c1 > 0 && st_c == p.c0) resetup = true;
    if (resetup) {
      if (st_tap < p.ksize * p.ksize) setup_rows();
    } else {
#pragma unroll
      for (int j = 0; j < GA; ++j) ap[j] += ainc[j];
    }
  };

  f32x4 acc[NT][MT];
#pragma unroll
  for (int i = 0; i < NT; ++i)
#pragma unroll
    for (int j = 0; j < MT; ++j) acc[i][j] = f32x4{0.f, 0.f, 0.f, 0.f};

  const int fr = lane & 15, fg = lane >> 4;
  float ln_s1[MT], ln_s2[MT];
#pragma unroll
  for (int j = 0; j < MT; ++j) { ln_s1[j] = 0.f; ln_s2[j] = 0.f; }
  float* ln_stat = reinterpret_cast<float*>(smem + NS * TILE);

  constexpr int G = GA + GB;
#pragma unroll
  for (int s0 = 0; s0 < NS - 1; ++s0)
    if (kt_begin + s0 < kt_end) stage(s0);
  int cur = 0;
  NR_STAMP_AT(1);
  for (int kt = kt_begin; kt < kt_end; ++kt) {
    if (kt + (NS - 2) < kt_end) nr_wait_vmcnt<(NS - 2) * G>(); else nr_wait_vmcnt<0>();
    __builtin_amdgcn_s_barrier();
    NR_STAMP_AT(4 + (kt - kt_begin));
    const bf16* sA = smem + cur * TILE;
    const bf16* sB = sA + BM * BK;
    bf16x8 wf[2][NT], xf[2][MT];
#pragma unroll
    for (int i = 0; i < NT; ++i) {
      const int row = wn * WN + i * 16 + fr;
      wf[0][i] = *(const bf16x8*)(sB + row * BK + ((fg ^ (row & 7)) << 3));
    }
#pragma unroll
    for (int j = 0; j < MT; ++j) {
      const int row = wm * WM + j * 16 + fr;
      xf[0][j] = *(const bf16x8*)(sA + row * BK + ((fg ^ (row & 7)) << 3));
    }
    __builtin_amdgcn_sched_barrier(0);
    {
      const int nxt = kt + NS - 1;
      int nb = cur + NS - 1; if (nb >= NS) nb -= NS;
      if (nxt < kt_end) stage(nb);
    }
    __builtin_amdgcn_sched_barrier(0);
#pragma unroll
    for (int i = 0; i < NT; ++i) {
      const int row = wn * WN + i * 16 + fr;
      wf[1][i] = *(const bf16x8*)(sB + row * BK + (((4 + fg) ^ (row & 7)) << 3));
    }
#pragma unroll
    for (int j = 0; j < MT; ++j) {
      const int row = wm * WM + j * 16 + fr;
      xf[1][j] = *(const bf16x8*)(sA + row * BK + (((4 + fg) ^ (row & 7)) << 3));
    }
#pragma unroll
    for (int ks = 0; ks < 2; ++ks)
#pragma unroll
      for (int i = 0; i < NT; ++i)
#pragma unroll
        for (int j = 0; j < MT; ++j)
          acc[i][j] = __builtin_amdgcn_mfma_f32_16x16x32_bf16(wf[ks][i], xf[ks][j], acc[i][j], 0, 0, 0);
    if constexpr (LNF) {
      const bf16x2 one2 = {(bf16)1.0f, (bf16)1.0f};
#pragma unroll
      for (int ks = 0; ks < 2; ++ks) {
        if (((2 * kt + ks) & (WGN - 1)) != wn) continue;
#pragma unroll
        for (int j = 0; j < MT; ++j)
#pragma unroll
          for (int e = 0; e < 4; ++e) {
            const bf16x2 pr = {xf[ks][j][2 * e], xf[ks][j][2 * e + 1]};
            ln_s2[j] = __builtin_amdgcn_fdot2_f32_bf16(pr, pr, ln_s2[j], false);
            ln_s1[j] = __builtin_amdgcn_fdot2_f32_bf16(pr, one2, ln_s1[j], false);
          }
      }
    }
    cur = cur + 1 == NS ? 0 : cur + 1;
  }
  NR_STAMP_AT(2);
  float ln_mu[MT], ln_rs[MT];
  if constexpr (LNF) {
#pragma unroll
    for (int j = 0; j < MT; ++j) {
      float a = ln_s1[j], b = ln_s2[j];
      a += __shfl_xor(a, 16, 64); b += __shfl_xor(b, 16, 64);
      a += __shfl_xor(a, 32, 64); b += __shfl_xor(b, 32, 64);
      if (fg == 0) {
        const int row = wm * WM + j * 16 + fr;
        ln_stat[(0 * WGN + wn) * BM + row] = a;
        ln_stat[(1 * WGN + wn) * BM + row] = b;
      }
    }
    __syncthreads();
#pragma unroll
    for (int j = 0; j < MT; ++j) {
      const int row = wm * WM + j * 16 + fr;
      float a = 0.f, b = 0.f;
#pragma unroll
      for (int w = 0; w < WGN; ++w) { a += ln_stat[(0 * WGN + w) * BM + row]; b += ln_stat[(1 * WGN + w) * BM + row]; }
      const float inv = 1.0f / (float)p.K;
      const float mu = a * inv;
      ln_mu[j] = mu;
      ln_rs[j] = rsqrtf(fmaxf(b * inv - mu * mu, 0.f) + p.ln_eps);
    }
#pragma unroll
    for (int i = 0; i < NT; ++i) {
      const int n = n0 + wn * WN + i * 16 + 4 * fg;
      const f32x4 cn = n < p.N ? *(const f32x4*)(p.ln_c + n) : f32x4{0.f, 0.f, 0.f, 0.f};
#pragma unroll
      for (int j = 0; j < MT; ++j)
#pragma unroll
        for (int r = 0; r < 4; ++r) acc[i][j][r] = ln_rs[j] * (acc[i][j][r] - ln_mu[j] * cn[r]);
    }
  }

  if (partial) {
    float* slab = partial + (size_t)slice * p.M * p.N;
#pragma unroll
    for (int j = 0; j < MT; ++j) {
      const int m = m0 + wm * WM + j * 16 + fr;
      if (m >= p.M) continue;
#pragma unroll
      for (int i = 0; i < NT; ++i) {
        const int n = n0 + wn * WN + i * 16 + 4 * fg;
        if (n >= p.N) continue;
        nr_store16f(slab + (size_t)m * p.N + n, acc[i][j]);
      }
    }
    return;
  }
  constexpr bool STAGED = (size_t)BM * BN * sizeof(float) <= (size_t)NS * TILE * sizeof(bf16);
  if constexpr (STAGED) {
    constexpr int NTH = 64 * NW;
    float* sC = reinterpret_cast<float*>(smem);
    __syncthreads();
    const int bno = p.geglu ? BN / 2 : BN;
#pragma unroll
    for (int j = 0; j < MT; ++j) {
      const int row = wm * WM + j * 16 + fr;
      if (!p.geglu) {
#pragma unroll
        for (int i = 0; i < NT; ++i) {
          const int c4 = ((wn * WN + i * 16) >> 2) + fg;
          *(f32x4*)(sC + row * BN + ((c4 ^ (row & 7)) << 2)) = acc[i][j];
        }
      } else {
        if constexpr (NT % 2 == 0) {
#pragma unroll
          for (int i = 0; i < NT; i += 2) {
            const int nv = n0 + wn * WN + i * 16 + 4 * fg;
            f32x4 v = acc[i][j], g = acc[i + 1][j];
            if (p.bias && nv < p.N) { v += *(const f32x4*)(p.bias + nv); g += *(const f32x4*)(p.bias + nv + 16); }
            f32x4 o;
#pragma unroll
            for (int e = 0; e < 4; ++e) o[e] = v[e] * gelu_erf_fast(g[e]);
            const int c4 = (((wn * WN + i * 16) >> 1) >> 2) + fg;
            *(f32x4*)(sC + row * BN + ((c4 ^ (row & 7)) << 2)) = o;
          }
        }
      }
    }
    __syncthreads();
    const int c8n = bno >> 3;
    const int nout = p.geglu ? p.N / 2 : p.N;
    const int nb0 = p.geglu ? n0 / 2 : n0;
    for (int idx = tid; idx < BM * c8n; idx += NTH) {
      const int row = idx / c8n, c8 = idx - row * c8n;
      const int m = m0 + row, n = nb0 + c8 * 8;
      if (m >= p.M || n >= nout) continue;
      f32x4 va = *(const f32x4*)(sC + row * BN + (((2 * c8) ^ (row & 7)) << 2));
      f32x4 vb = *(const f32x4*)(sC + row * BN + (((2 * c8 + 1) ^ (row & 7)) << 2));
      if (!p.geglu) {
        if (p.bias) { va += *(const f32x4*)(p.bias + n); vb += *(const f32x4*)(p.bias + n + 4); }
        if (p.rowvec) {
          const float* rv = p.rowvec + nr_rowvec_row(p, m) + n;
          va += *(const f32x4*)rv; vb += *(const f32x4*)(rv + 4);
        }
        va *= p.out_scale; vb *= p.out_scale;
        if (p.act == 1) {
#pragma unroll
          for (int e = 0; e < 4; ++e) { va[e] = quick_gelu_f(va[e]); vb[e] = quick_gelu_f(vb[e]); }
        }
        if (p.res) {
          const bf16x8 r = *(const bf16x8*)(p.res + (size_t)m * p.ldr + n);
#pragma unroll
          for (int e = 0; e < 4; ++e) { va[e] += (float)r[e]; vb[e] += (float)r[4 + e]; }
        }
      }
      bf16x8 o;
#pragma unroll
      for (int e = 0; e < 4; ++e) { o[e] = (bf16)va[e]; o[4 + e] = (bf16)vb[e]; }
      nr_store16(p.out + (size_t)m * p.ldo + n, o);
    }
#ifdef NR_STAMP
    asm volatile("s_waitcnt vmcnt(0)" ::: "memory");
#endif
    NR_STAMP_AT(3);
    NR_STAMP_RT(45);
    return;
  }
#pragma unroll
  for (int j = 0; j < MT; ++j) {
    const int m = m0 + wm * WM + j * 16 + fr;
    if (m >= p.M) continue;
    const float* rv = p.rowvec ? p.rowvec + nr_rowvec_row(p, m) : nullptr;
    if (!p.geglu) {
#pragma unroll
      for (int i = 0; i < NT; ++i) {
        const int n = n0 + wn * WN + i * 16 + 4 * fg;
        if (n >= p.N) continue;
        f32x4 v = acc[i][j];
        if (p.bias) { const f32x4 b = *(const f32x4*)(p.bias + n); v += b; }
        if (rv) { const f32x4 t = *(const f32x4*)(rv + n); v += t; }
        v *= p.out_scale;
        if (p.act == 1) {
#pragma unroll
          for (int e = 0; e < 4; ++e) v[e] = quick_gelu_f(v[e]);
        }
        if (p.res) {
          const bf16x4 r = *(const bf16x4*)(p.res + (size_t)m * p.ldr + n);
#pragma unroll
          for (int e = 0; e < 4; ++e) v[e] += (float)r[e];
        }
        bf16x4 o;
#pragma unroll
        for (int e = 0; e < 4; ++e) o[e] = (bf16)v[e];
        nr_store8(p.out + (size_t)m * p.ldo + n, o);
      }
    } else {
      if constexpr (NT % 2 == 0) {
#pragma unroll
        for (int i = 0; i < NT; i += 2) {
          const int nv = n0 + wn * WN + i * 16 + 4 * fg;
          if (nv >= p.N) continue;
          const int ng = nv + 16;
          f32x4 v = acc[i][j], g = acc[i + 1][j];
          if (p.bias) {
            v += *(const f32x4*)(p.bias + nv);
            g += *(const f32x4*)(p.bias + ng);
          }
          const int oc = ((n0 + wn * WN + i * 16) >> 1) + 4 * fg;
          bf16x4 o;
#pragma unroll
          for (int e = 0; e < 4; ++e) o[e] = (bf16)(v[e] * gelu_erf_fast(g[e]));
          nr_store8(p.out + (size_t)m * p.ldo + oc, o);
        }
      }
    }
  }
}

__global__ __launch_bounds__(256) void splitk_reduce_kernel(NrGemmParams p_arg, int splitk, const float* __restrict__ partial) {
  const NrGemmParams p = nr_pin_params(p_arg);
  const long long idx = (long long)blockIdx.x * 256 + threadIdx.x;
  const int n4 = p.N >> 2;
  if (idx >= (long long)p.M * n4) return;
  const int m = (int)(idx / n4);
  const int n = (int)(idx - (long long)m * n4) << 2;
  const size_t slab = (size_t)p.M * p.N;
  const float* src = partial + (size_t)m * p.N + n;
  f32x4 v = *(const f32x4*)src;
  for (int s = 1; s < splitk; ++s) v += *(const f32x4*)(src + s * slab);
  if (p.bias) v += *(const f32x4*)(p.bias + n);
  if (p.rowvec) v += *(const f32x4*)(p.rowvec + nr_rowvec_row(p, m) + n);
  v *= p.out_scale;
  if (p.act == 1) {
#pragma unroll
    for (int e = 0; e < 4; ++e) v[e] = quick_gelu_f(v[e]);
  }
  if (p.res) {
    const bf16x4 r = *(const bf16x4*)(p.res + (size_t)m * p.ldr + n);
#pragma unroll
    for (int e = 0; e < 4; ++e) v[e] += (float)r[e];
  }
  bf16x4 o;
#pragma unroll
  for (int e = 0; e < 4; ++e) o[e] = (bf16)v[e];
  nr_store8(p.out + (size_t)m * p.ldo + n, o);
}

typedef TiledPlan Plan;

Plan choose_plan(const NrGemmParams& p) {
  auto nblk = [&](int bm, int bn) { return (long long)((p.M + bm - 1) / bm) * ((p.N + bn - 1) / bn); };
  const int nk = p.K / 64;
  Plan pl{};
  pl.splitk = 1; pl.stages = 2; pl.waves = 4;
  if (!p.geglu && p.M <= 1024 && nk >= 128 && p.N % 160 == 0) {
    pl.bm = 128; pl.bn = 160; pl.splitk = nk >= 300 ? 16 : 8;
    return pl;
  }
  if (!p.geglu && p.ksize == 3 && p.M <= 2048 && nk >= 128 && p.N % 160 == 0) {
    pl.bm = 128; pl.bn = 160; pl.splitk = 4;
    return pl;
  }
  if (!p.geglu && p.ksize == 3 && p.M <= 8192 && p.N % 160 == 0 && p.N < 960 && nk >= 64 && nblk(128, 160) >= 128 && nblk(128, 160) < 512) {
    pl.bm = 128; pl.bn = 160; pl.splitk = 2;
    return pl;
  }
  if (!p.geglu && p.ksize == 1 && p.M <= 2048 && p.M > 512 && nk >= 96 && p.N % 160 == 0) {
    pl.bm = 128; pl.bn = 160; pl.splitk = 4;
    return pl;
  }
  static const bool t64x160_rule = env_not_0("NR_IGEMM_T64X160");
  if (t64x160_rule && p.ksize == 1 && !p.geglu && p.N % 160 == 0 && p.M > 512 && nk >= 16 && nk <= 48 && nblk(64, 160) >= 128 && nblk(64, 160) <= 256) {
    pl.bm = 64; pl.bn = 160; pl.stages = 3;
    return pl;
  }
  const bool n128 = p.N % 128 == 0 || p.N >= 960;
  if (!p.geglu && p.N % 160 == 0 && p.N < 960 && p.N % 128 != 0 && nk >= 20 && nblk(128, 160) >= 256) { pl.bm = 128; pl.bn = 160; }
  else if (n128 && nblk(128, 128) >= 400) { pl.bm = 128; pl.bn = 128; pl.waves = 8; }
  else if (nblk(128, 64) >= 512 || (nblk(128, 64) >= 256 && nk > 32)) { pl.bm = 128; pl.bn = 64; pl.waves = nk <= 32 ? 8 : 4; }
  else if (nblk(64, 64) >= 256 && nk <= 96) { pl.bm = 64; pl.bn = 64; }
  else if (p.M >= 1024 && nblk(128, 64) >= 64) { pl.bm = 128; pl.bn = 64; }
  else { pl.bm = 64; pl.bn = 64; }
  static const bool smallm_rule = env_not_0("NR_IGEMM_SMALLM");
  static const bool wide_rule = env_not_0("NR_IGEMM_WIDE");
  static const bool rowwave_rule = env_not_0("NR_IGEMM_ROWWAVE");
  if (smallm_rule && p.ksize == 1 && p.M <= 512 && nk >= 8) {
    pl.bm = 64; pl.bn = p.geglu ? 64 : 32; pl.waves = 4; pl.stages = 4;
    if (p.geglu && p.N >= 8192 && p.M >= 256) { pl.bm = 128; pl.bn = 128; pl.waves = 8; pl.stages = 2; }
    if (rowwave_rule && p.geglu && p.N >= 8192 && p.N % 160 == 0 && p.M > 256 && nblk(128, 160) <= 256) {
      pl.bm = 128; pl.bn = 160; pl.waves = 41; pl.stages = p.ln_c ? 3 : 4;
    }
    else if (!p.geglu && nk >= 96 && !p.ln_c) { pl.bm = 64; pl.bn = 64; pl.stages = 2; pl.splitk = 4; return pl; }
    else if (wide_rule && !p.geglu && nblk(64, 32) > 640 && nblk(128, 64) >= 192) { pl.bm = 128; pl.bn = 64; pl.waves = 8; pl.stages = 4; }
  }
  if (!p.geglu) {
    const long long tiles = nblk(pl.bm, pl.bn);
    const int cap_m = p.M >= 8192 ? 2 : (p.M >= 2048 ? 4 : 8);
    const int min_tiles = p.M <= 1024 ? 8 : 16;
    if (tiles < 512 && nk >= 4 * min_tiles) {
      int s_ = (int)((1280 + tiles - 1) / tiles);
      if (s_ > nk / min_tiles) s_ = nk / min_tiles;
      if (s_ > cap_m) s_ = cap_m;
      if (s_ < 1) s_ = 1;
      pl.splitk = s_;
    }
  }
  return pl;
}

inline NrGemmParams plan_view(const NrGemmParams& p) {
  NrGemmParams q = p;
  q.M = nr_plan_rows(p);
  return q;
}

typedef void (*igemm_kern_t)(NrGemmParams, int, float*, int);

template <int BM, int BN, int NS, int WGM, int WGN>
int launch_cfg(const NrGemmParams& p, unsigned grid, const Plan& pl, float* partial, int m_fast, hipStream_t stream) {
  size_t shm = (size_t)NS * (BM + BN) * 64 * sizeof(bf16);
  constexpr bool LN_OK = (NS == 2 && BM <= 128 && BN <= 128) || (NS == 4 && (BM * BN <= 64 * 64 || (BM == 128 && BN == 64))) ||
                         (BM == 128 && BN == 160 && WGN == 1 && NS <= 4) ||
                         (BM == 64 && BN == 160 && NS <= 3);
  igemm_kern_t k = nullptr;
  int ki = 0;
  if (p.ln_c) {
    if constexpr (LN_OK) { k = igemm_bf16_kernel<BM, BN, NS, WGM, WGN, true>; shm += (size_t)2 * WGN * BM * sizeof(float); }
    else return 9;
  } else {
    k = !pl.adma ? igemm_bf16_kernel<BM, BN, NS, WGM, WGN, false, false> : igemm_bf16_kernel<BM, BN, NS, WGM, WGN, false, true>;
    ki = 1 + pl.adma;
    if constexpr (NS <= 4) {
      if (pl.lin) {
        k = !pl.adma ? igemm_bf16_kernel<BM, BN, NS, WGM, WGN, false, false, true> : igemm_bf16_kernel<BM, BN, NS, WGM, WGN, false, true, true>;
        ki += 2;
      }
    }
  }
  static unsigned long long attr_done[5] = {};
  (void)nr_lds_opt_in(attr_done[ki], {(const void*)k}, shm);
  hipLaunchKernelGGL(k, dim3(grid), dim3(64 * WGM * WGN), shm, stream, p, pl.splitk, partial, m_fast);
  return 0;
}

template <int BM, int BN, int WGM, int WGN>
int launch_tile(const NrGemmParams& p, unsigned grid, const Plan& pl, float* partial, int m_fast, hipStream_t stream) {
  constexpr size_t STAGE = (size_t)(BM + BN) * 64 * sizeof(bf16);
  constexpr bool FITS4 = 4 * STAGE <= 160 * 1024;
  if (pl.stages <= 2) return launch_cfg<BM, BN, 2, WGM, WGN>(p, grid, pl, partial, m_fast, stream);
  if (pl.stages == 3 || !FITS4) return launch_cfg<BM, BN, 3, WGM, WGN>(p, grid, pl, partial, m_fast, stream);
  if (pl.stages <= 4 || BM * BN > 64 * 64) return launch_cfg<BM, BN, 4, WGM, WGN>(p, grid, pl, partial, m_fast, stream);
  if (pl.stages <= 6) return launch_cfg<BM, BN, 6, WGM, WGN>(p, grid, pl, partial, m_fast, stream);
  return launch_cfg<BM, BN, 8, WGM, WGN>(p, grid, pl, partial, m_fast, stream);
}

void apply_override(const NrGemmParams& p, Plan& pl, int& m_fast) {
  const char* e = getenv("NR_IGEMM_FORCE");
  if (!e) return;
  if (const char* f = getenv("NR_IGEMM_FORCE_MAXM")) if (p.M > atoi(f)) return;
  if (const char* f = getenv("NR_IGEMM_FORCE_MINM")) if (p.M < atoi(f)) return;
  if (const char* f = getenv("NR_IGEMM_FORCE_KS")) if (p.ksize != atoi(f)) return;
  if (const char* f = getenv("NR_IGEMM_FORCE_N")) if (p.N != atoi(f)) return;
  if (const char* f = getenv("NR_IGEMM_FORCE_K")) if (p.K != atoi(f)) return;
  int bm = -1, bn = -1, sk = -1, st = -1, ord = -1, wv = -1;
  sscanf(e, "%d,%d,%d,%d,%d,%d", &bm, &bn, &sk, &st, &ord, &wv);
  if (bm > 0 && bn > 0) {
    const bool ok = (bm == 128 && (bn == 160 || bn == 128 || bn == 64)) || (bm == 64 && (bn == 64 || bn == 32 || bn == 160)) || (bm == 256 && (bn == 128 || bn == 160));
    if (ok && !(p.geglu && ((bn == 160 && !(bm == 128 && wv == 41)) || bn == 32))) { pl.bm = bm; pl.bn = bn; }
  }
  if (wv == 4 || wv == 8) pl.waves = wv;
  if (pl.bm == 256 && pl.bn == 128 && wv != 4) pl.waves = 8;
  if (pl.bn == 160 || pl.bm == 64) pl.waves = 4;
  if (wv == 41 && pl.bm == 128 && pl.bn == 160) pl.waves = 41;
  if (sk > 0 && !p.geglu) { const int nk = p.K / 64; pl.splitk = sk > nk ? nk : sk; }
  if (st >= 2 && st <= 8) pl.stages = st;
  if (ord >= 0) m_fast = ord;
}

int tile_order(double w_elems, double a_elems, int ntm, int ntn) {
  static const bool grouped = env_not_0("NR_IGEMM_GROUPED");
  static const double grouped_minw = getenv("NR_IGEMM_GROUPED_MINW") ? atof(getenv("NR_IGEMM_GROUPED_MINW")) : 3.0e6;
  if (grouped && ntm >= 8 && ntn >= 4 && w_elems >= grouped_minw) return 8;
  return w_elems > a_elems ? 1 : 0;
}

int route(const NrGemmParams& p, NrGemmRoute* r, bool packed_ok) {
  std::memset(r, 0, sizeof(*r));
  r->weight_layout = p.tap_inner ? NR_W_TAP_INNER : NR_W_ROWMAJOR;
  const int Cin = p.c0 + p.c1;
  if (packed_ok && smallm_plan(p, &r->smallm)) { r->cls = NR_GEMM_SMALLM; r->weight_layout = p.w8 ? NR_W_FRAGMAJOR_E4M3 : NR_W_FRAGMAJOR; return 0; }
  if (packed_ok && lin160_plan(p, &r->lin160)) { r->cls = NR_GEMM_LIN160; r->weight_layout = r->lin160.form == 4 ? NR_W_LIN128Q : NR_W_LIN160; return 0; }
  if (p.K == p.ksize * p.ksize * Cin && rowpanel_plan(p, &r->rowpanel)) { r->cls = NR_GEMM_ROWPANEL; return 0; }
  const double w_elems = (double)p.N * p.K;
  if (g8p_plan(p, &r->g8p)) {
    r->cls = NR_GEMM_G8P;
    r->m_fast = tile_order(w_elems, (double)p.M * Cin, (p.M + 255) / 256, (p.N + 64 * r->g8p.nt - 1) / (64 * r->g8p.nt));
    return 0;
  }
  r->cls = NR_GEMM_TILED;
  if (p.K % 64 != 0 || Cin % 64 != 0 || p.N % 32 != 0) return 1;
  if (p.a1 && (p.c0 % 64 != 0)) return 2;
  if (p.K != p.ksize * p.ksize * Cin) return 3;
  if (p.ksize != 1 && p.ksize != 3) return 4;
  if (p.tap_inner && (p.ksize != 3 || p.stride != 1 || p.ups || p.pad_tl0 || p.a1)) return 5;
  Plan& pl = r->tiled;
  pl = choose_plan(plan_view(p));
  const double a_elems = (double)p.M * Cin * (p.ksize == 3 ? (p.stride == 2 ? 4.0 : (p.ups ? 0.25 : 1.0)) : 1.0);
  r->m_fast = tile_order(w_elems, a_elems, (p.M + pl.bm - 1) / pl.bm, (p.N + pl.bn - 1) / pl.bn);
  apply_override(p, pl, r->m_fast);
  if (p.ln_c) {
    if (p.ksize != 1 || p.a1 || p.out_f32) return 8;
    pl.splitk = 1;
    if (pl.bn == 32) pl.bn = 64;
    const bool t64x160 = pl.bm == 64 && pl.bn == 160;
    if (!(pl.stages == 4 && (pl.bm * pl.bn <= 64 * 64 || (pl.bm == 128 && pl.bn == 64))) && pl.waves != 41 && !(t64x160 && pl.stages <= 3)) pl.stages = 2;
    if (pl.bm > 128) { pl.bm = 128; pl.bn = 128; pl.waves = 8; }
    if (pl.bn > 128 && !(pl.bm == 128 && pl.bn == 160 && pl.waves == 41) && !t64x160) { pl.bm = 128; pl.bn = 128; pl.waves = 8; }
    if (pl.waves == 41 && pl.stages > 4) pl.stages = 4;
  }
  if (p.out_f32) {
    if (p.geglu) return 7;
    pl.splitk = 1;
  }
  static const int adma_min = getenv("NR_IGEMM_ADMA_MINK") ? atoi(getenv("NR_IGEMM_ADMA_MINK")) : 24;
  static const bool lin_on = env_not_0("NR_IGEMM_LIN");
  pl.adma = (p.K / 64) / (pl.splitk > 1 ? pl.splitk : 1) >= adma_min;
  pl.lin = lin_on && p.ksize == 1 && !p.a1 && p.c1 == 0;
  r->ws_bytes = pl.splitk > 1 ? (size_t)pl.splitk * p.M * p.N * sizeof(float) : 0;
  return 0;
}

int launch_tiled(const NrGemmParams& p, const Plan& pl, int m_fast, float* workspace, hipStream_t stream) {
  if (pl.splitk < 1 || pl.splitk > p.K / 64 || ((p.ln_c || p.out_f32) && pl.splitk != 1)) return 9;
  if (pl.splitk > 1 && !workspace) return 6;
  float* partial = p.out_f32 ? p.out_f32 : (pl.splitk > 1 ? workspace : nullptr);
  const unsigned grid = (unsigned)(((p.M + pl.bm - 1) / pl.bm) * ((p.N + pl.bn - 1) / pl.bn) * pl.splitk);
  int rc;
  if (pl.bm == 256 && pl.bn == 160) rc = launch_tile<256, 160, 2, 2>(p, grid, pl, partial, m_fast, stream);
  else if (pl.bm == 256 && pl.waves == 4) rc = launch_tile<256, 128, 2, 2>(p, grid, pl, partial, m_fast, stream);
  else if (pl.bm == 256) rc = launch_tile<256, 128, 4, 2>(p, grid, pl, partial, m_fast, stream);
  else if (pl.bm == 128 && pl.bn == 160 && pl.waves == 41)
    rc = pl.stages <= 3 ? launch_cfg<128, 160, 3, 4, 1>(p, grid, pl, partial, m_fast, stream)
                        : launch_cfg<128, 160, 4, 4, 1>(p, grid, pl, partial, m_fast, stream);
  else if (pl.bm == 128 && pl.bn == 160) rc = launch_tile<128, 160, 2, 2>(p, grid, pl, partial, m_fast, stream);
  else if (pl.bm == 128 && pl.bn == 128 && pl.waves == 8) rc = launch_tile<128, 128, 2, 4>(p, grid, pl, partial, m_fast, stream);
  else if (pl.bm == 128 && pl.bn == 128) rc = launch_tile<128, 128, 2, 2>(p, grid, pl, partial, m_fast, stream);
  else if (pl.bm == 128 && pl.bn == 64 && pl.waves == 8) rc = launch_tile<128, 64, 4, 2>(p, grid, pl, partial, m_fast, stream);
  else if (pl.bm == 128 && pl.bn == 64) rc = launch_tile<128, 64, 2, 2>(p, grid, pl, partial, m_fast, stream);
  else if (pl.bm == 64 && pl.bn == 160) rc = launch_tile<64, 160, 2, 2>(p, grid, pl, partial, m_fast, stream);
  else if (pl.bm == 64 && pl.bn == 32) rc = launch_tile<64, 32, 2, 2>(p, grid, pl, partial, m_fast, stream);
  else if (pl.bm == 64 && pl.bn == 64) rc = launch_tile<64, 64, 2, 2>(p, grid, pl, partial, m_fast, stream);
  else rc = 9;
  if (rc) return rc;
  if (pl.splitk > 1) {
    const long long total = (long long)p.M * (p.N / 4);
    hipLaunchKernelGGL(splitk_reduce_kernel, dim3((unsigned)((total + 255) / 256)), dim3(256), 0, stream, p, pl.splitk,
                       (const float*)partial);
  }
  return 0;
}

}

extern "C" int nr_gemm_route(const NrGemmParams* pp, NrGemmRoute* r) { return route(*pp, r, true); }
extern "C" int nr_gemm_route_rowmajor(const NrGemmParams* pp, NrGemmRoute* r) { return route(*pp, r, false); }

extern "C" int nr_launch_gemm(const NrGemmParams* pp, const NrGemmRoute* r, const bf16* packed_w, float* ws, hipStream_t stream) {
  switch (r->cls) {
    case NR_GEMM_SMALLM: return nr_launch_smallm(pp, &r->smallm, packed_w, r->weight_layout, stream);
    case NR_GEMM_LIN160: return nr_launch_lin160(pp, &r->lin160, packed_w, stream);
    case NR_GEMM_ROWPANEL: return nr_launch_rowpanel(pp, &r->rowpanel, stream);
    case NR_GEMM_G8P: return nr_launch_g8p(pp, &r->g8p, r->m_fast, stream);
    case NR_GEMM_TILED: return launch_tiled(*pp, r->tiled, r->m_fast, ws, stream);
  }
  return 9;
}

extern "C" size_t nr_gemm_packed_bytes(int layout, int N, int K) {
  switch (layout) {
    case NR_W_FRAGMAJOR: return (N % 16 == 0 && K % 32 == 0) ? (size_t)N * K * sizeof(bf16) : 0;
    case NR_W_FRAGMAJOR_E4M3: return (N > 0 && K > 0 && N % 16 == 0 && K % 64 == 0) ? (size_t)N * K + (size_t)N * sizeof(float) : 0;
    case NR_W_LIN160: return nr_lin160_stream_bytes(N, K);
    case NR_W_LIN128Q: return nr_lin128q_stream_bytes(N, K);
  }
  return 0;
}
extern "C" int nr_launch_gemm_w_pack(int layout, const bf16* w, int N, int K, bf16* dst, hipStream_t stream) {
  switch (layout) {
    case NR_W_FRAGMAJOR: return nr_launch_smallm_w_pack(w, dst, N, K, stream);
    case NR_W_FRAGMAJOR_E4M3: return nr_launch_smallm_w8_pack(w, dst, N, K, stream);
    case NR_W_LIN160: return nr_launch_lin160_w_pack(w, N, K, dst, stream);
    case NR_W_LIN128Q: return nr_launch_lin128q_w_pack(w, N, K, dst, stream);
  }
  return 1;
}

#ifdef NR_STAMP
extern "C" int nr_stamp_read(void* dst, size_t bytes, int clear) { return nr_stamp_read_buf(nr_stamp_buf, dst, bytes, clear); }
#endif
```

neurons_amd/ops.py:

```python
import torch

from . import _lib


def _ptr(t):
    return None if t is None else t.data_ptr()


def _stream():
    return torch.cuda.current_stream().cuda_stream


def _chk_bf16(*ts):
    for t in ts:
        if t is not None:
            assert t.is_cuda and t.dtype == torch.bfloat16 and t.is_contiguous(), (t.dtype, t.shape)


def _chk_f32(*ts):
    for t in ts:
        if t is not None:
            assert t.is_cuda and t.dtype == torch.float32 and t.is_contiguous(), (t.dtype, t.shape)


# ... 32 lines not shown
    _lib.load().nr_g8p_set_mode(int(mode))


def g8p_phases(n):
    _lib.load().nr_g8p_set_phases(int(n))


def ff_waves(n):
    _lib.load().nr_ff_set_waves(int(n))


def _ln_fold(w, gamma, beta, bias=None):
    wf = w.float()
    ws = (wf * gamma.float()[None]).to(torch.bfloat16).contiguous()
    c = ws.float().sum(dim=1).contiguous()
    b = (wf.double() @ beta.double()).float()
    if bias is not None:
        b = b + bias.float()
    return ws, c, b.contiguous()


def ln_gemm(a, w, gamma, beta, bias=None, res=None, eps=1e-5, act=0, geglu=False):
    _chk_bf16(a, res)
    M, K = a.shape
    if geglu:
        w, bias = geglu_permute(w, bias)
    N = w.shape[0]
    ws, c, b = _ln_fold(w, gamma, beta, bias)
    No = N // 2 if geglu else N
    out = torch.empty(M, No, dtype=torch.bfloat16, device=a.device)
    lib = _lib.load()
    _lib.check(lib.nr_op_ln_gemm(_stream(), _ptr(a), K, _ptr(ws), _ptr(c), _ptr(b), float(eps), _ptr(res), No, _ptr(out), No, M, N, K, 1 if geglu else 0,
                                 int(act)))
    return out


def gemm_ex(a, w, bias=None, ln=None, eps=1e-5, rowvec=None, rowvec_div=1, rowvec_mod=0, res=None, act=0, out_scale=1.0):
    _chk_bf16(a, res)
    _chk_f32(rowvec)
    M, K = a.shape
    N = w.shape[0]
    if ln is not None:
        ws, ln_c, b = _ln_fold(w, ln[0], ln[1], bias)
    else:
        ws, ln_c, b = w.to(torch.bfloat16).contiguous(), None, None if bias is None else bias.float().contiguous()
    out = torch.empty(M, N, dtype=torch.bfloat16, device=a.device)
    lib = _lib.load()
    _lib.check(lib.nr_op_gemm_ex(_stream(), _ptr(a), K, _ptr(ws), _ptr(b), _ptr(ln_c), float(eps), _ptr(rowvec), int(rowvec_div),
                                 int(rowvec_mod), 0 if rowvec is None else rowvec.shape[1], _ptr(res), N, _ptr(out), N, M, N, K, 0, int(act),
                                 float(out_scale)))
    return out


def geglu_permute(w, b):
    inner = w.shape[0] // 2
    n = torch.arange(2 * inner)
    q, j = n // 32, n % 32
    src = torch.where(j < 16, q * 16 + j, inner + q * 16 + (j - 16))
    return w[src].contiguous(), (None if b is None else b[src].contiguous())


def conv3x3(x0, w, bias=None, x1=None, stride=1, ups=False, rowvec=None, rowvec_div=1, res=None, tap_inner=False):
    _chk_bf16(x0, x1, w, res)
    _chk_f32(bias, rowvec)
    nimg, H, W, c0 = x0.shape
    if tap_inner:
        if x1 is not None or stride != 1 or ups or c0 % 64 != 0:
            raise ValueError("tap_inner: stride 1, no upsample, one source, Cin % 64 == 0")
        Cout = w.shape[0]
        wt = w.reshape(Cout, 9, c0 // 64, 64).permute(0, 2, 1, 3).contiguous()
        out = torch.empty(nimg, H, W, Cout, dtype=torch.bfloat16, device=x0.device)
        _lib.check(_lib.load().nr_op_conv3x3_tap_inner(_stream(), _ptr(x0), c0, nimg, H, W, _ptr(wt), _ptr(bias), _ptr(rowvec), rowvec_div,
                                                        _ptr(res), _ptr(out), Cout))
        return out
    c1 = 0 if x1 is None else x1.shape[3]
    Cout = w.shape[0]
    OH, OW = (2 * H, 2 * W) if ups else (H, W)
    if stride == 2:
        OH, OW = (OH - 1) // 2 + 1, (OW - 1) // 2 + 1
    out = torch.empty(nimg, OH, OW, Cout, dtype=torch.bfloat16, device=x0.device)
    lib = _lib.load()
    _lib.check(lib.nr_op_conv3x3(_stream(), _ptr(x0), c0, _ptr(x1), c1, nimg, H, W, stride, 1 if ups else 0, _ptr(w),
                                 _ptr(bias), _ptr(rowvec), rowvec_div, _ptr(res), _ptr(out), Cout))
    return out


def condembed_pack(w):
    Cout, Cin = w.shape[:2]
    K = 9 * Cin
    KS = (K + 31) // 32
    wk = torch.zeros(Cout, KS * 32, dtype=torch.float32, device=w.device)
    wk[:, :K] = w.float().permute(0, 2, 3, 1).reshape(Cout, K)
    return wk.reshape(Cout // 16, 16, KS, 4, 8).permute(0, 2, 3, 1, 4).contiguous().to(torch.bfloat16)


def condembed_conv(x, w, bias, stride=1, silu=True):
    _chk_bf16(x)
    _chk_f32(bias)
    nimg, H, W, Cin = x.shape
    Cout = w.shape[0]
    OH, OW = ((H - 1) // 2 + 1, (W - 1) // 2 + 1) if stride == 2 else (H, W)
    wfm = condembed_pack(w)
    out = torch.empty(nimg, OH, OW, Cout, dtype=torch.bfloat16, device=x.device)
    _lib.check(_lib.load().nr_op_condembed_conv(_stream(), _ptr(x), nimg, H, W, Cin, stride, _ptr(wfm), _ptr(bias), Cout, 1 if silu else 0,
                                                _ptr(out)))
    return out


def condembed_in(cond, mask, w, bias, frames=None):
    import ctypes as C
    _chk_f32(cond, mask, bias)
    b, c0, F, H, W = cond.shape
    Cout = w.shape[0]
    frames = list(range(F)) if frames is None else [int(f) for f in frames]
    wT = w.float().reshape(Cout, -1).t().contiguous()
    fm = (C.c_int32 * len(frames))(*frames)
    out = torch.empty(b * len(frames), H, W, Cout, dtype=torch.bfloat16, device=cond.device)
    _lib.check(_lib.load().nr_op_condembed_in(_stream(), _ptr(cond), _ptr(mask), c0, b, F, H, W, fm, len(frames), _ptr(wT), _ptr(bias), Cout,
                                              _ptr(out)))
    return out


def groupnorm(x0, gamma, beta, groups=32, eps=1e-5, silu=False, x1=None):
    _chk_bf16(x0, x1)
    _chk_f32(gamma, beta)
    nimg, H, W, c0 = x0.shape
    c1 = 0 if x1 is None else x1.shape[3]
    out = torch.empty(nimg, H, W, c0 + c1, dtype=torch.bfloat16, device=x0.device)
    ws = torch.empty(nimg * (H * W) * groups * 2 + 64, dtype=torch.float32, device=x0.device)
    lib = _lib.load()
    _lib.check(lib.nr_op_groupnorm(_stream(), _ptr(x0), c0, _ptr(x1), c1, nimg, H * W, groups, _ptr(gamma), _ptr(beta),
                                   eps, 1 if silu else 0, _ptr(ws), _ptr(out)))
    return out


def layernorm(x, gamma, beta, eps=1e-5, pe=None, pe_hw=1, pe_F=1):
    _chk_bf16(x)
    _chk_f32(gamma, beta, pe)
    M, Cc = x.shape
    out = torch.empty_like(x)
    lib = _lib.load()
    _lib.check(lib.nr_op_layernorm(_stream(), _ptr(x), _ptr(out), M, Cc, _ptr(gamma), _ptr(beta), eps, _ptr(pe), pe_hw, pe_F))
    return out


def _attn_out(out, shape, like):
    if out is None:
        return torch.empty(*shape, dtype=torch.bfloat16, device=like.device)
    _chk_bf16(out)
    if tuple(out.shape) != tuple(shape) or out.device != like.device:
        raise ValueError(f"out: expected a bf16 tensor of shape {tuple(shape)} on {like.device}, got {tuple(out.shape)} on {out.device}")
    return out


def attention_self(qkv, heads, fp8=False, causal=False, out=None):
    _chk_bf16(qkv)
    nimg, L, C3 = qkv.shape
    Cc = C3 // 3
    out = _attn_out(out, (nimg, L, Cc), qkv)
    lib = _lib.load()
    _lib.check(lib.nr_op_attention(_stream(), (8 if fp8 else 0) | (16 if causal else 0), _ptr(qkv), None, _ptr(out), nimg, L, L, Cc, heads, 1, 1))
    return out


def attention_cross(q, kv, heads, kv_div, fp8=False, out=None):
    _chk_bf16(q, kv)
# ... 214 lines not shown
```

Before: 20.32 frames/s.

## Decompose nearest-upsample 3x3 conv into four 2x2 phase convolutions

```diff
diff --git a/include/neurons_amd.h b/include/neurons_amd.h
--- a/include/neurons_amd.h
+++ b/include/neurons_amd.h
@@ -196,6 +196,9 @@
 nr_status nr_op_conv3x3(nr_stream stream, const void* x0_dev, int32_t c0, const void* x1_dev, int32_t c1, int32_t nimg,
                         int32_t H, int32_t W, int32_t stride, int32_t ups, const void* w_dev, const float* bias_dev,
                         const float* rowvec_dev, int32_t rowvec_div, const void* res_dev, void* out_dev, int32_t Cout);
+nr_status nr_op_conv3x3_ups_phase(nr_stream stream, const void* x_dev, int32_t Cin, int32_t nimg, int32_t H, int32_t W, const void* wp_dev,
+                                  const float* bias_dev, void* out_dev, int32_t Cout);
+nr_status nr_ups_phase_weights(const float* w_tap_host, int32_t Cout, int32_t Cin, void* out_host);
 nr_status nr_op_condembed_in(nr_stream stream, const float* cond_dev, const float* mask_dev, int32_t c0, int32_t nsrc, int32_t F, int32_t H,
                              int32_t W, const int32_t* fmap, int32_t nframes, const float* w_dev, const float* bias_dev, int32_t Cout,
                              void* out_dev);
diff --git a/neurons_amd/_lib.py b/neurons_amd/_lib.py
--- a/neurons_amd/_lib.py
+++ b/neurons_amd/_lib.py
@@ -117,6 +117,8 @@
     "nr_op_gemm_ex": (_I32, [_VP, _VP, _I32, _VP, _VP, _VP, C.c_float, _VP, _I32, _I32, _I32, _VP, _I32, _VP, _I32, _I32, _I32, _I32, _I32, _I32,
                              C.c_float]),
     "nr_op_conv3x3": (_I32, [_VP, _VP, _I32, _VP, _I32, _I32, _I32, _I32, _I32, _I32, _VP, _VP, _VP, _I32, _VP, _VP, _I32]),
+    "nr_op_conv3x3_ups_phase": (_I32, [_VP, _VP, _I32, _I32, _I32, _I32, _VP, _VP, _VP, _I32]),
+    "nr_ups_phase_weights": (_I32, [_VP, _I32, _I32, _VP]),
     "nr_op_condembed_in": (_I32, [_VP, _VP, _VP, _I32, _I32, _I32, _I32, _I32, C.POINTER(_I32), _I32, _VP, _VP, _I32, _VP]),
     "nr_op_condembed_conv": (_I32, [_VP, _VP, _I32, _I32, _I32, _I32, _I32, _VP, _VP, _I32, _I32, _VP]),
     "nr_op_conv3x3_tap_inner": (_I32, [_VP, _VP, _I32, _I32, _I32, _I32, _VP, _VP, _VP, _I32, _VP, _VP, _I32]),
diff --git a/neurons_amd/csrc/common.h b/neurons_amd/csrc/common.h
--- a/neurons_amd/csrc/common.h
+++ b/neurons_amd/csrc/common.h
@@ -182,7 +182,7 @@
   nr_conv_out_hw(H, W, ksize, stride, ups, &p.OH, &p.OW);
   p.ksize = ksize; p.stride = stride; p.ups = ups;
   p.w = w;
-  p.M = nimg * p.OH * p.OW; p.N = N; p.K = ksize * ksize * (p.c0 + p.c1);
+  p.M = nimg * p.OH * p.OW; p.N = N; p.K = (ups == 2 ? 4 : ksize * ksize) * (p.c0 + p.c1);
   p.bias = bias; p.rowvec_div = 1;
   p.res = res; p.ldr = ldr;
   p.out = out; p.ldo = ldo; p.out_scale = 1.f;
diff --git a/neurons_amd/csrc/engine.h b/neurons_amd/csrc/engine.h
--- a/neurons_amd/csrc/engine.h
+++ b/neurons_amd/csrc/engine.h
@@ -56,6 +56,22 @@
   if ((u & 0x7fffffffu) > 0x7f800000u) return 0x7fc0;
   u += 0x7fffu + ((u >> 16) & 1u);
   return (uint16_t)(u >> 16);
+}
+
+inline void nr_ups_phase_pack(const float* w, size_t so, size_t sc, size_t sk, int Cout, int Cin, uint16_t* out) {
+  static const int lo[2][2] = {{0, 1}, {0, 2}}, hi[2][2] = {{0, 2}, {1, 2}};
+  for (int ph = 0; ph < 4; ++ph)
+    for (int o = 0; o < Cout; ++o)
+      for (int t = 0; t < 4; ++t) {
+        const int py = ph >> 1, px = ph & 1, a = t >> 1, b = t & 1;
+        uint16_t* dst = out + (((size_t)ph * Cout + o) * 4 + t) * Cin;
+        for (int c = 0; c < Cin; ++c) {
+          float acc = 0.f;
+          for (int ky = lo[py][a]; ky <= hi[py][a]; ++ky)
+            for (int kx = lo[px][b]; kx <= hi[px][b]; ++kx) acc += w[o * so + c * sc + (size_t)(3 * ky + kx) * sk];
+          dst[c] = f2bf_host(acc);
+        }
+      }
 }
 
 template <class... A>
@@ -215,6 +231,7 @@
   const bf16* w_geglu(const std::string& key, int inner, int K);
   const float* b_geglu(const std::string& key, int inner);
   const bf16* w_conv3(const std::string& key, int Cout, int Cin, bool tap_inner = false);
+  const bf16* w_conv3_ups_phase(const std::string& key, int Cout, int Cin);
   const float* w_conv_in(const std::string& key, int Cout, int Cin);
   const bf16* w_condembed(const std::string& key, int Cout, int Cin);
   const float* w_f32_sum(const std::string& a, const std::string& b, int64_t n);
@@ -277,6 +294,7 @@
   int cond_frames[64] = {0};
   bool cfg_dup = false;
   bool attn_fp8 = false;
+  int ups_phase_mode = -1;
   bool w8 = false;
   IO io = nre::new_io();
   int n_res = 0;
@@ -338,6 +356,7 @@
   };
   Act conv(const Act& x0, const Act* x1, const bf16* w, int Cout, int ksize, int stride, int ups, const GemmOpt& o);
   Act linear(const Act& x, const bf16* w, int N, const GemmOpt& o) { return conv(x, nullptr, w, N, 1, 1, 0, o); }
+  Act upsample_conv(const Act& x, const std::string& wkey, int Cout, const GemmOpt& o);
   Act linear_wb(const Act& x, const std::string& key, int N, const Act* res = nullptr, Act* out = nullptr);
   void gemm_raw(const bf16* a, int lda, const bf16* w, int M, int N, int K, const float* bias, bf16* out, int ldo, float* out32, const char* what);
   Act groupnorm(const Act& x0, const Act* x1, const std::string& prefix, float eps, int silu);
diff --git a/neurons_amd/csrc/engine_layers.hip b/neurons_amd/csrc/engine_layers.hip
--- a/neurons_amd/csrc/engine_layers.hip
+++ b/neurons_amd/csrc/engine_layers.hip
@@ -67,6 +67,7 @@
 void nr_net::begin_plan() {
   ctx_persist.clear(); ops.clear(); ctx_ops.clear(); op_meta.clear(); taps.clear(); arena.reset(); parena.reset();
   ctx_dirty = true;
+  { const char* e = getenv("NR_UPS_PHASE"); ups_phase_mode = (e && e[0]) ? (e[0] != '0' ? 1 : 0) : -1; }
   temb_slots.clear(); temb_total = 0; temb_all = nullptr;
   n_res = 0; res_shapes.clear();
   t_dev = new_scratch<float>(NR_MAX_BATCH);
@@ -115,7 +116,8 @@
   LAUNCH_OK(nr_gemm_route(&p, &r));
   const bf16* wk = dry ? reinterpret_cast<const bf16*>(uintptr_t(16)) : wts.w_layout(w, Cout, p.K, r.weight_layout);
   const double in_elems = (double)x0.rows() * (p.c0 + p.c1);
-  const double bytes = 2.0 * (in_elems + (double)p.N * p.K + (double)p.M * outC + (o.res ? (double)p.M * outC : 0.0));
+  const double w_elems = (double)p.N * p.K * (ups == 2 ? 4 : 1);
+  const double bytes = 2.0 * (in_elems + w_elems + (double)p.M * outC + (o.res ? (double)p.M * outC : 0.0));
   const bool l160 = r.cls == NR_GEMM_LIN160;
   const std::string d = l160 ? descf("%s M=%d N=%d K=%d res=%d geglu=%d ln=%d", r.lin160.form == 4 ? "lin160 panel" : "lin160", p.M, p.N, p.K, o.res ? 1 : 0, p.geglu, p.ln_c ? 1 : 0)
                              : descf("igemm ks=%d s=%d ups=%d M=%d N=%d K=%d geglu=%d res=%d%s", ksize, stride, ups, p.M, p.N, p.K, p.geglu, o.res ? 1 : 0,
@@ -126,6 +128,19 @@
   if (ws) last_op_launches(2);
   op_tap(l160 ? "lin160" : (ksize == 3 ? "conv3" : (p.ln_c ? "lngemm" : "gemm")), out);
   return out;
+}
+
+static bool nr_ups_phase_rule(long long M, int N, int Cin) {
+  (void)N;
+  return Cin >= 1280 ? M >= 2048 : M >= 32768;
+}
+Act nr_net::upsample_conv(const Act& x, const std::string& wkey, int Cout, const GemmOpt& o) {
+  const int Cin = x.C;
+  const long long M = det_rows((long long)x.nimg * x.H * x.W * 4);
+  const bool eligible = Cin % 64 == 0 && Cout % 32 == 0 && !o.res && !o.rowvec && !o.geglu && !o.ln_c && !o.tap_inner && !o.pad_tl0;
+  const bool phase = eligible && ups_phase_mode != 0 && (ups_phase_mode == 1 || nr_ups_phase_rule(M, Cout, Cin));
+  if (phase) return conv(x, nullptr, wts.w_conv3_ups_phase(wkey, Cout, Cin), Cout, 3, 1, 2, o);
+  return conv(x, nullptr, wts.w_conv3(wkey, Cout, Cin), Cout, 3, 1, 1, o);
 }
 
 Act nr_net::linear_wb(const Act& x, const std::string& key, int N, const Act* res, Act* out) {
diff --git a/neurons_amd/csrc/engine_nets.hip b/neurons_amd/csrc/engine_nets.hip
--- a/neurons_amd/csrc/engine_nets.hip
+++ b/neurons_amd/csrc/engine_nets.hip
@@ -122,7 +122,7 @@
     if (b.up) {
       const std::string up = bp + "." + std::to_string(sub) + ".conv";
       GemmOpt o; o.bias = wts.w_f32(up + ".bias", b.Cout);
-      x = conv(x, nullptr, wts.w_conv3(up + ".weight", b.Cout, b.Cout), b.Cout, 3, 1, 1, o);
+      x = upsample_conv(x, up + ".weight", b.Cout, o);
       tap(bp + "." + std::to_string(sub), x);
     }
   }
@@ -166,7 +166,7 @@
     for (int j = 0; j < cfg.layers_per_block + 1; ++j) x = resnet(x, nullptr, up + ".block." + std::to_string(j), Co);
     if (lev != 0) {
       GemmOpt o; o.bias = wts.w_f32(up + ".upsample.conv.bias", Co);
-      x = conv(x, nullptr, wts.w_conv3(up + ".upsample.conv.weight", Co, Co), Co, 3, 1, 1, o);
+      x = upsample_conv(x, up + ".upsample.conv.weight", Co, o);
       tap(up + ".upsample", x);
     }
   }
@@ -595,7 +595,7 @@
     }
     if (i != L - 1) {
       GemmOpt o; o.bias = wts.w_f32(bp + ".upsamplers.0.conv.bias", Cout);
-      x = conv(x, nullptr, wts.w_conv3(bp + ".upsamplers.0.conv.weight", Cout, Cout), Cout, 3, 1, 1, o);
+      x = upsample_conv(x, bp + ".upsamplers.0.conv.weight", Cout, o);
       tap(bp + ".upsamplers.0", x);
     }
   }
diff --git a/neurons_amd/csrc/engine_ops.hip b/neurons_amd/csrc/engine_ops.hip
--- a/neurons_amd/csrc/engine_ops.hip
+++ b/neurons_amd/csrc/engine_ops.hip
@@ -112,6 +112,21 @@
                                   Cout, (bf16*)out, Cout);
   p.rowvec = rowvec; p.rowvec_div = rowvec_div > 0 ? rowvec_div : 1; p.rowvec_ld = Cout;
   op_gemm(p, (hipStream_t)stream);
+  NR_CATCH
+}
+
+extern "C" nr_status nr_op_conv3x3_ups_phase(nr_stream stream, const void* x, int32_t Cin, int32_t nimg, int32_t H, int32_t W, const void* wp,
+                                             const float* bias, void* out, int32_t Cout) {
+  NR_TRY
+  if (!x || !wp || !out) throw NrError(NR_ERR_ARG, "null argument");
+  NrGemmParams p = nr_gemm_params((const bf16*)x, Cin, Cin, nullptr, 0, 0, nimg, H, W, 3, 1, 2, (const bf16*)wp, Cout, bias, nullptr, 0, (bf16*)out, Cout);
+  op_gemm(p, (hipStream_t)stream);
+  NR_CATCH
+}
+extern "C" nr_status nr_ups_phase_weights(const float* w_tap, int32_t Cout, int32_t Cin, void* out) {
+  NR_TRY
+  if (!w_tap || !out || Cout < 1 || Cin < 1) throw NrError(NR_ERR_ARG, "bad argument");
+  nr_ups_phase_pack(w_tap, (size_t)9 * Cin, 1, (size_t)Cin, Cout, Cin, (uint16_t*)out);
   NR_CATCH
 }
 
diff --git a/neurons_amd/csrc/engine_weights.hip b/neurons_amd/csrc/engine_weights.hip
--- a/neurons_amd/csrc/engine_weights.hip
+++ b/neurons_amd/csrc/engine_weights.hip
@@ -343,6 +343,11 @@
         }
   });
 }
+const bf16* WeightStore::w_conv3_ups_phase(const std::string& key, int Cout, int Cin) {
+  return (const bf16*)convert<uint16_t>("conv3up:", key, {Cout, Cin, 3, 3}, (size_t)16 * Cout * Cin, [&](const float* s, uint16_t* h) {
+    nr_ups_phase_pack(s, (size_t)Cin * 9, 9, 1, Cout, Cin, h);
+  });
+}
 const float* WeightStore::w_conv_in(const std::string& key, int Cout, int Cin) {
   return convert<float>("convin:", key, {Cout, Cin, 3, 3}, (size_t)Cin * 9 * Cout, [&](const float* s, float* h) {
     for (int o = 0; o < Cout; ++o)
diff --git a/neurons_amd/csrc/gemm.hip b/neurons_amd/csrc/gemm.hip
--- a/neurons_amd/csrc/gemm.hip
+++ b/neurons_amd/csrc/gemm.hip
@@ -13,10 +13,12 @@
 #define NR_STAMP_AT(slot) NR_STAMP_PUT(nr_stamp_buf, slot)
 #define NR_STAMP_RT(slot) NR_STAMP_PUT_RT(nr_stamp_buf, slot)
 
-template <int BM, int BN, int NS, int WGM, int WGN, bool LNF = false, bool ADMA = false, bool LIN = LNF>
+template <int BM, int BN, int NS, int WGM, int WGN, bool LNF = false, bool ADMA = false, bool LIN = LNF, bool PH = false>
 __global__ __launch_bounds__(64 * WGM * WGN, (LNF && WGM * WGN == 8) ? 4 : 1) void igemm_bf16_kernel(NrGemmParams p_arg, int splitk, float* partial, int m_fast) {
   NrGemmParams p = nr_pin_params(p_arg);
   if constexpr (LIN) { p.ksize = 1; p.stride = 1; p.ups = 0; p.a1 = nullptr; p.c1 = 0; p.tap_inner = 0; p.pad_tl0 = 0; }
+  static_assert(!PH || (!LIN && !LNF), "the phase form is a conv");
+  if constexpr (PH) { p.ksize = 3; p.stride = 1; p.ups = 2; p.a1 = nullptr; p.c1 = 0; p.tap_inner = 0; p.pad_tl0 = 0; p.geglu = 0; p.rowvec = nullptr; p.res = nullptr; }
   splitk = nr_pin(splitk); partial = nr_pin(partial); m_fast = nr_pin(m_fast);
   constexpr int BK = 64;
   constexpr int NW = WGM * WGN;
@@ -34,7 +36,9 @@
   NR_STAMP_RT(44);
   const int wm = wave / WGN, wn = wave % WGN;
   const int ntn = (p.N + BN - 1) / BN;
-  const int ntm = (p.M + BM - 1) / BM;
+  const int Mrows = PH ? p.M >> 2 : p.M;
+  const int ntmp = (Mrows + BM - 1) / BM;
+  const int ntm = PH ? 4 * ntmp : ntmp;
   int bid;
   {
     const int nwg = gridDim.x, orig = blockIdx.x;
@@ -53,7 +57,17 @@
     bn = nr_fdiv_small(r, gsz);
     bm = first + r - bn * gsz;
   } else if (m_fast) { bn = nr_fdiv_small(bid, ntm); bm = bid - bn * ntm; } else { bm = nr_fdiv_small(bid, ntn); bn = bid - bm * ntn; }
+  const int phase = PH ? nr_fdiv_small(bm, ntmp) : 0;
+  if constexpr (PH) bm -= phase * ntmp;
+  const int ph_py = phase >> 1, ph_px = phase & 1;
   const int m0 = bm * BM, n0 = bn * BN;
+  auto ph_out_row = [&](int r) {
+    const int hw = p.H * p.W;
+    const int n = nr_fdiv_small(r, hw);
+    const int q = r - n * hw;
+    const int y = nr_fdiv_small(q, p.W), x = q - y * p.W;
+    return (n * p.OH + 2 * y + ph_py) * p.OW + 2 * x + ph_px;
+  };
   NR_STAMP_AT(40);
   const int lr = lane >> 3;
   const int lp = lane & 7;
@@ -66,9 +80,14 @@
 #pragma unroll
   for (int j = 0; j < GA; ++j) {
     const int m = m0 + 8 * (wave * GA + j) + lr;
-    a_ok[j] = m < p.M;
+    a_ok[j] = m < Mrows;
     const int mm = a_ok[j] ? m : 0;
-    if (p.ksize == 1) {
+    if constexpr (PH) {
+      const int hw = p.H * p.W;
+      const int n = nr_fdiv_small(mm, hw);
+      const int r = mm - n * hw;
+      a_pix[j] = n; a_oy[j] = nr_fdiv_small(r, p.W); a_ox[j] = r - a_oy[j] * p.W;
+    } else if (p.ksize == 1) {
       a_pix[j] = mm; a_oy[j] = 0; a_ox[j] = 0;
     } else {
       const int ohw = p.OH * p.OW;
@@ -113,7 +132,7 @@
     for (int j = 0; j < GB; ++j) {
       const int n = n0 + 8 * (wave * GB + j) + lr;
       const bool ok = n < p.N;
-      wp[j] = ok ? p.w + (size_t)n * p.K + kbase + lchunk : zsrc;
+      wp[j] = ok ? p.w + ((size_t)phase * p.N + n) * p.K + kbase + lchunk : zsrc;
       winc[j] = ok ? BK : 0;
     }
   }
@@ -132,7 +151,17 @@
     const bf16* src; int ld;
     if (st_c < p.c0) { src = p.a0 + st_c; ld = p.lda0; } else { src = p.a1 + (st_c - p.c0); ld = p.lda1; }
     src += lchunk;
-    if (p.ksize == 1) {
+    if constexpr (PH) {
+      const int dy = (st_tap >> 1) + ph_py - 1, dx = (st_tap & 1) + ph_px - 1;
+#pragma unroll
+      for (int j = 0; j < GA; ++j) {
+        const int iy = a_oy[j] + dy, ix = a_ox[j] + dx;
+        const bool ok = a_ok[j] && iy >= 0 && iy < p.H && ix >= 0 && ix < p.W;
+        const size_t pix = ((size_t)a_pix[j] * p.H + iy) * p.W + ix;
+        ap[j] = ok ? src + pix * ld : zsrc;
+        ainc[j] = ok ? BK : 0;
+      }
+    } else if (p.ksize == 1) {
 #pragma unroll
       for (int j = 0; j < GA; ++j) {
         ap[j] = a_ok[j] ? src + (size_t)a_pix[j] * ld : zsrc;
@@ -185,7 +214,7 @@
     if (st_c == Cin) { st_c = 0; st_tap += 1; resetup = true; }
     else if (p.c1 > 0 && st_c == p.c0) resetup = true;
     if (resetup) {
-      if (st_tap < p.ksize * p.ksize) setup_rows();
+      if (st_tap < (PH ? 4 : p.ksize * p.ksize)) setup_rows();
     } else {
 #pragma unroll
       for (int j = 0; j < GA; ++j) ap[j] += ainc[j];
@@ -310,12 +339,13 @@
 #pragma unroll
     for (int j = 0; j < MT; ++j) {
       const int m = m0 + wm * WM + j * 16 + fr;
-      if (m >= p.M) continue;
+      if (m >= Mrows) continue;
+      const int ms = PH ? phase * Mrows + m : m;
 #pragma unroll
       for (int i = 0; i < NT; ++i) {
         const int n = n0 + wn * WN + i * 16 + 4 * fg;
         if (n >= p.N) continue;
-        nr_store16f(slab + (size_t)m * p.N + n, acc[i][j]);
+        nr_store16f(slab + (size_t)ms * p.N + n, acc[i][j]);
       }
     }
     return;
@@ -358,7 +388,7 @@
     for (int idx = tid; idx < BM * c8n; idx += NTH) {
       const int row = idx / c8n, c8 = idx - row * c8n;
       const int m = m0 + row, n = nb0 + c8 * 8;
-      if (m >= p.M || n >= nout) continue;
+      if (m >= Mrows || n >= nout) continue;
       f32x4 va = *(const f32x4*)(sC + row * BN + (((2 * c8) ^ (row & 7)) << 2));
       f32x4 vb = *(const f32x4*)(sC + row * BN + (((2 * c8 + 1) ^ (row & 7)) << 2));
       if (!p.geglu) {
@@ -381,7 +411,7 @@
       bf16x8 o;
 #pragma unroll
       for (int e = 0; e < 4; ++e) { o[e] = (bf16)va[e]; o[4 + e] = (bf16)vb[e]; }
-      nr_store16(p.out + (size_t)m * p.ldo + n, o);
+      nr_store16(p.out + (size_t)(PH ? ph_out_row(m) : m) * p.ldo + n, o);
     }
 #ifdef NR_STAMP
     asm volatile("s_waitcnt vmcnt(0)" ::: "memory");
@@ -393,7 +423,8 @@
 #pragma unroll
   for (int j = 0; j < MT; ++j) {
     const int m = m0 + wm * WM + j * 16 + fr;
-    if (m >= p.M) continue;
+    if (m >= Mrows) continue;
+    const size_t mo = PH ? ph_out_row(m) : m;
     const float* rv = p.rowvec ? p.rowvec + nr_rowvec_row(p, m) : nullptr;
     if (!p.geglu) {
 #pragma unroll
@@ -416,7 +447,7 @@
         bf16x4 o;
 #pragma unroll
         for (int e = 0; e < 4; ++e) o[e] = (bf16)v[e];
-        nr_store8(p.out + (size_t)m * p.ldo + n, o);
+        nr_store8(p.out + mo * p.ldo + n, o);
       }
     } else {
       if constexpr (NT % 2 == 0) {
@@ -434,13 +465,14 @@
           bf16x4 o;
 #pragma unroll
           for (int e = 0; e < 4; ++e) o[e] = (bf16)(v[e] * gelu_erf_fast(g[e]));
-          nr_store8(p.out + (size_t)m * p.ldo + oc, o);
+          nr_store8(p.out + mo * p.ldo + oc, o);
         }
       }
     }
   }
 }
 
+template <bool PH>
 __global__ __launch_bounds__(256) void splitk_reduce_kernel(NrGemmParams p_arg, int splitk, const float* __restrict__ partial) {
   const NrGemmParams p = nr_pin_params(p_arg);
   const long long idx = (long long)blockIdx.x * 256 + threadIdx.x;
@@ -467,16 +499,54 @@
   bf16x4 o;
 #pragma unroll
   for (int e = 0; e < 4; ++e) o[e] = (bf16)v[e];
-  nr_store8(p.out + (size_t)m * p.ldo + n, o);
+  size_t mo = (size_t)m;
+  if constexpr (PH) {
+    const int Mp = p.M >> 2, hw = p.H * p.W;
+    const int phase = m / Mp, r = m - phase * Mp;
+    const int img = r / hw, q = r - img * hw;
+    const int y = q / p.W, x = q - y * p.W;
+    mo = (size_t)(img * p.OH + 2 * y + (phase >> 1)) * p.OW + 2 * x + (phase & 1);
+  }
+  nr_store8(p.out + mo * p.ldo + n, o);
 }
 
 typedef TiledPlan Plan;
 
+constexpr bool phase_tile(int bm, int bn, int waves) {
+  return (bm == 128 && bn == 160 && waves == 4) || (bm == 128 && bn == 128 && waves == 8) || (bm == 128 && bn == 64 && waves == 4) ||
+         (bm == 64 && bn == 64 && waves == 4) || (bm == 256 && bn == 128 && waves == 8);
+}
+inline long long row_tiles(const NrGemmParams& p, int bm) { return p.ups == 2 ? 4ll * ((p.M / 4 + bm - 1) / bm) : (p.M + bm - 1) / bm; }
+
+Plan choose_plan_phase(const NrGemmParams& p) {
+  auto nblk = [&](int bm, int bn) { return row_tiles(p, bm) * ((p.N + bn - 1) / bn); };
+  const int nk = p.K / 64;
+  Plan pl{};
+  pl.splitk = 1; pl.stages = 2; pl.waves = 4;
+  if (p.N % 160 == 0) {
+    pl.bm = 128; pl.bn = 160;
+    if (p.M <= 2048 && nk >= 64) { pl.splitk = 4; return pl; }
+  } else {
+    const bool n128 = p.N % 128 == 0 || p.N >= 960;
+    if (n128 && nblk(128, 128) >= 400) { pl.bm = 128; pl.bn = 128; pl.waves = 8; }
+    else if (nblk(128, 64) >= 256) { pl.bm = 128; pl.bn = 64; }
+    else { pl.bm = 64; pl.bn = 64; }
+  }
+  const long long tiles = nblk(pl.bm, pl.bn);
+  if (tiles < 512 && nk >= 64) {
+    int s_ = (int)((1024 + tiles - 1) / tiles);
+    if (s_ > nk / 16) s_ = nk / 16;
+    if (s_ > 4) s_ = 4;
+    pl.splitk = s_ < 1 ? 1 : s_;
+  }
+  return pl;
+}
 Plan choose_plan(const NrGemmParams& p) {
   auto nblk = [&](int bm, int bn) { return (long long)((p.M + bm - 1) / bm) * ((p.N + bn - 1) / bn); };
   const int nk = p.K / 64;
   Plan pl{};
   pl.splitk = 1; pl.stages = 2; pl.waves = 4;
+  if (p.ups == 2) return choose_plan_phase(p);
   if (!p.geglu && p.M <= 1024 && nk >= 128 && p.N % 160 == 0) {
     pl.bm = 128; pl.bn = 160; pl.splitk = nk >= 300 ? 16 : 8;
     return pl;
@@ -551,6 +621,11 @@
   if (p.ln_c) {
     if constexpr (LN_OK) { k = igemm_bf16_kernel<BM, BN, NS, WGM, WGN, true>; shm += (size_t)2 * WGN * BM * sizeof(float); }
     else return 9;
+  } else if (p.ups == 2) {
+    if constexpr (phase_tile(BM, BN, WGM * WGN) && NS == 2) {
+      k = !pl.adma ? igemm_bf16_kernel<BM, BN, NS, WGM, WGN, false, false, false, true> : igemm_bf16_kernel<BM, BN, NS, WGM, WGN, false, true, false, true>;
+      ki = 5 + pl.adma;
+    } else return 9;
   } else {
     k = !pl.adma ? igemm_bf16_kernel<BM, BN, NS, WGM, WGN, false, false> : igemm_bf16_kernel<BM, BN, NS, WGM, WGN, false, true>;
     ki = 1 + pl.adma;
@@ -561,7 +636,7 @@
       }
     }
   }
-  static unsigned long long attr_done[5] = {};
+  static unsigned long long attr_done[7] = {};
   (void)nr_lds_opt_in(attr_done[ki], {(const void*)k}, shm);
   hipLaunchKernelGGL(k, dim3(grid), dim3(64 * WGM * WGN), shm, stream, p, pl.splitk, partial, m_fast);
   return 0;
@@ -612,11 +687,17 @@
   std::memset(r, 0, sizeof(*r));
   r->weight_layout = p.tap_inner ? NR_W_TAP_INNER : NR_W_ROWMAJOR;
   const int Cin = p.c0 + p.c1;
-  if (packed_ok && smallm_plan(p, &r->smallm)) { r->cls = NR_GEMM_SMALLM; r->weight_layout = p.w8 ? NR_W_FRAGMAJOR_E4M3 : NR_W_FRAGMAJOR; return 0; }
-  if (packed_ok && lin160_plan(p, &r->lin160)) { r->cls = NR_GEMM_LIN160; r->weight_layout = r->lin160.form == 4 ? NR_W_LIN128Q : NR_W_LIN160; return 0; }
-  if (p.K == p.ksize * p.ksize * Cin && rowpanel_plan(p, &r->rowpanel)) { r->cls = NR_GEMM_ROWPANEL; return 0; }
+  const bool phase = p.ups == 2;
+  if (phase) {
+    r->cls = NR_GEMM_TILED;
+    if (p.ksize != 3 || p.stride != 1 || p.a1 || p.c1 || p.tap_inner || p.pad_tl0 || p.geglu || p.ln_c || p.out_f32 || p.res || p.rowvec) return 10;
+    if (p.H < 1 || p.W < 1 || p.OH != 2 * p.H || p.OW != 2 * p.W || p.M < 4 || p.M % (p.OH * p.OW) != 0) return 11;
+  } else if (p.ups != 0 && p.ups != 1) return 11;
+  if (!phase && packed_ok && smallm_plan(p, &r->smallm)) { r->cls = NR_GEMM_SMALLM; r->weight_layout = p.w8 ? NR_W_FRAGMAJOR_E4M3 : NR_W_FRAGMAJOR; return 0; }
+  if (!phase && packed_ok && lin160_plan(p, &r->lin160)) { r->cls = NR_GEMM_LIN160; r->weight_layout = r->lin160.form == 4 ? NR_W_LIN128Q : NR_W_LIN160; return 0; }
+  if (!phase && p.K == p.ksize * p.ksize * Cin && rowpanel_plan(p, &r->rowpanel)) { r->cls = NR_GEMM_ROWPANEL; return 0; }
   const double w_elems = (double)p.N * p.K;
-  if (g8p_plan(p, &r->g8p)) {
+  if (!phase && g8p_plan(p, &r->g8p)) {
     r->cls = NR_GEMM_G8P;
     r->m_fast = tile_order(w_elems, (double)p.M * Cin, (p.M + 255) / 256, (p.N + 64 * r->g8p.nt - 1) / (64 * r->g8p.nt));
     return 0;
@@ -624,14 +705,21 @@
   r->cls = NR_GEMM_TILED;
   if (p.K % 64 != 0 || Cin % 64 != 0 || p.N % 32 != 0) return 1;
   if (p.a1 && (p.c0 % 64 != 0)) return 2;
-  if (p.K != p.ksize * p.ksize * Cin) return 3;
+  if (p.K != (phase ? 4 : p.ksize * p.ksize) * Cin) return 3;
   if (p.ksize != 1 && p.ksize != 3) return 4;
   if (p.tap_inner && (p.ksize != 3 || p.stride != 1 || p.ups || p.pad_tl0 || p.a1)) return 5;
   Plan& pl = r->tiled;
   pl = choose_plan(plan_view(p));
   const double a_elems = (double)p.M * Cin * (p.ksize == 3 ? (p.stride == 2 ? 4.0 : (p.ups ? 0.25 : 1.0)) : 1.0);
-  r->m_fast = tile_order(w_elems, a_elems, (p.M + pl.bm - 1) / pl.bm, (p.N + pl.bn - 1) / pl.bn);
+  const int ntm1 = (int)(phase ? row_tiles(p, pl.bm) / 4 : row_tiles(p, pl.bm));
+  r->m_fast = tile_order(w_elems, a_elems, ntm1, (p.N + pl.bn - 1) / pl.bn);
   apply_override(p, pl, r->m_fast);
+  if (phase) {
+    pl.stages = 2;
+    if (pl.bm == 256 || (pl.bm == 128 && pl.bn == 128)) pl.waves = 8; else pl.waves = 4;
+    if (!phase_tile(pl.bm, pl.bn, pl.waves)) { pl.bm = 128; pl.bn = 128; pl.waves = 8; }
+    if (r->m_fast >= 2 && (row_tiles(p, pl.bm) / 4) % r->m_fast != 0) r->m_fast = w_elems > a_elems ? 1 : 0;
+  }
   if (p.ln_c) {
     if (p.ksize != 1 || p.a1 || p.out_f32) return 8;
     pl.splitk = 1;
@@ -658,7 +746,7 @@
   if (pl.splitk < 1 || pl.splitk > p.K / 64 || ((p.ln_c || p.out_f32) && pl.splitk != 1)) return 9;
   if (pl.splitk > 1 && !workspace) return 6;
   float* partial = p.out_f32 ? p.out_f32 : (pl.splitk > 1 ? workspace : nullptr);
-  const unsigned grid = (unsigned)(((p.M + pl.bm - 1) / pl.bm) * ((p.N + pl.bn - 1) / pl.bn) * pl.splitk);
+  const unsigned grid = (unsigned)(row_tiles(p, pl.bm) * ((p.N + pl.bn - 1) / pl.bn) * pl.splitk);
   int rc;
   if (pl.bm == 256 && pl.bn == 160) rc = launch_tile<256, 160, 2, 2>(p, grid, pl, partial, m_fast, stream);
   else if (pl.bm == 256 && pl.waves == 4) rc = launch_tile<256, 128, 2, 2>(p, grid, pl, partial, m_fast, stream);
@@ -678,8 +766,8 @@
   if (rc) return rc;
   if (pl.splitk > 1) {
     const long long total = (long long)p.M * (p.N / 4);
-    hipLaunchKernelGGL(splitk_reduce_kernel, dim3((unsigned)((total + 255) / 256)), dim3(256), 0, stream, p, pl.splitk,
-                       (const float*)partial);
+    hipLaunchKernelGGL(p.ups == 2 ? splitk_reduce_kernel<true> : splitk_reduce_kernel<false>, dim3((unsigned)((total + 255) / 256)), dim3(256), 0, stream, p,
+                       pl.splitk, (const float*)partial);
   }
   return 0;
 }
diff --git a/neurons_amd/ops.py b/neurons_amd/ops.py
--- a/neurons_amd/ops.py
+++ b/neurons_amd/ops.py
@@ -138,6 +138,25 @@
     lib = _lib.load()
     _lib.check(lib.nr_op_conv3x3(_stream(), _ptr(x0), c0, _ptr(x1), c1, nimg, H, W, stride, 1 if ups else 0, _ptr(w),
                                  _ptr(bias), _ptr(rowvec), rowvec_div, _ptr(res), _ptr(out), Cout))
+    return out
+
+
+def ups_phase_weights(w_tap):
+    Cout, _, _, Cin = w_tap.shape
+    src = w_tap.detach().to("cpu", torch.float32).contiguous()
+    out = torch.empty(4, Cout, 4, Cin, dtype=torch.bfloat16)
+    _lib.check(_lib.load().nr_ups_phase_weights(src.data_ptr(), Cout, Cin, out.data_ptr()))
+    return out
+
+
+def conv3x3_ups_phase(x, w_tap, bias=None):
+    _chk_bf16(x)
+    _chk_f32(bias)
+    nimg, H, W, Cin = x.shape
+    Cout = w_tap.shape[0]
+    wp = ups_phase_weights(w_tap).to(x.device)
+    out = torch.empty(nimg, 2 * H, 2 * W, Cout, dtype=torch.bfloat16, device=x.device)
+    _lib.check(_lib.load().nr_op_conv3x3_ups_phase(_stream(), _ptr(x), Cin, nimg, H, W, _ptr(wp), _ptr(bias), _ptr(out), Cout))
     return out
 
 
```

Result: faster. 20.80 frames/s (median of 6 runs) (+2.4%).
